# Qualcomm-AI-research/transformer-quantization

Hardware: AMD Instinct MI355X
Metric: M elems/sec fake-quant fwd (BERT-base act tensor); achieved HBM GB/s vs peak (higher is better)
Workload: dtype f32; 1 GPU; BERT-base W8A8 per-tensor asym 8-bit activation fake-quant, running-minmax calibrated, fixed-range fwd, hidden [1024,512,768] bf16 per GPU (BASELINE configs[1]); storage_dtype=bf16, parallelism=dp1 (independent shards, no data-path collective)

## Files before the change

### include/tq_hip.h

```cpp
#ifndef TQ_HIP_H
#define TQ_HIP_H

#include <stddef.h>
#include <stdint.h>

#ifdef __cplusplus
extern "C" {
#endif

#define TQ_ABI_VERSION 2

enum { TQ_F32 = 0, TQ_BF16 = 1, TQ_F16 = 2 };
enum { TQ_IDX_NONE = 0, TQ_IDX_F32 = 1, TQ_IDX_I8 = 2, TQ_IDX_U8 = 3, TQ_IDX_I16 = 4,
       TQ_IDX_I32 = 5, TQ_IDX_I8_M128 = 6  };
enum { TQ_OK = 0, TQ_EINVAL = -1, TQ_ELAUNCH = -2, TQ_EWORKSPACE = -3, TQ_EUNSUPPORTED = -4 };
enum { TQ_EST_CURRENT = 0, TQ_EST_ALL = 1, TQ_EST_RUNNING = 2 };
enum { TQ_ADA_SIGMOID = 0, TQ_ADA_HARD_SIGMOID = 1, TQ_ADA_SIGMOID_TEMP = 2 };

typedef void* tq_stream_t;

typedef struct tq_quantizer {
  const float*   delta;
  const float*   zero_float;
  const uint8_t* signed_flag;
// ... 8 lines not shown
int tq_abi_version(void);
const char* tq_last_error(void);

int tq_fake_quant_fwd(const void* x, void* y, void* idx, int idx_dtype, uint64_t n, int dtype,
                      const tq_quantizer* q, tq_stream_t stream);

typedef struct tq_fq_item {
  const void*  x;
  void*        y;
  uint64_t     n;
  tq_quantizer q;
} tq_fq_item;
int tq_fake_quant_multi_fwd(const tq_fq_item* items, uint32_t n_items, int dtype, tq_stream_t stream);

int tq_affine_fake_quant_fwd(const void* x, const float* w, const float* b, void* y,
                             int8_t* y_idx ,
                             uint64_t n, uint64_t d, int dtype, const tq_quantizer* q, tq_stream_t stream);

int tq_residual_layernorm_quant_fwd(const void* dense_out, const void* residual, void* y,
                                    int8_t* y_idx ,
                                    uint64_t rows, uint64_t d, int dtype,
                                    const tq_quantizer* q_dense, const tq_quantizer* q_sum,
                                    const float* ln_weight, const float* ln_bias, float ln_eps,
                                    const tq_quantizer* q_out, tq_stream_t stream);

int tq_residual_layernorm_quant_axis_fwd(const void* dense_out, const void* residual, void* y,
                                         int8_t* y_idx ,
                                         uint64_t rows, uint64_t d, int dtype,
                                         const tq_quantizer* q_dense, const tq_quantizer* q_sum,
                                         const float* ln_weight, const float* ln_bias, float ln_eps,
                                         const tq_quantizer* q_out, tq_stream_t stream);

int tq_residual_nonorm_quant_fwd(const void* dense_out, const void* residual, void* y, int8_t* y_idx,
                                 uint64_t rows, uint64_t d, int dtype, const tq_quantizer* q_dense,
                                 const tq_quantizer* q_sum, const float* weight, const float* bias,
                                 const tq_quantizer* q_out, tq_stream_t stream);

int tq_embeddings_layernorm_quant_fwd(const float* word_table, uint64_t word_rows, const int64_t* word_ids,
                                      const float* type_table, uint64_t type_rows, const int64_t* type_ids,
                                      const float* pos_table, uint64_t pos_rows, const int64_t* pos_ids, float* y,
                                      int8_t* y_idx , uint64_t rows, uint64_t d,
                                      const tq_quantizer* q_sum1, const tq_quantizer* q_sum2, const float* ln_weight,
                                      const float* ln_bias, float ln_eps, const tq_quantizer* q_out,
                                      int32_t* bad_ids , tq_stream_t stream);

enum { TQ_ACT_NONE = 0, TQ_ACT_RELU = 1, TQ_ACT_GELU = 2, TQ_ACT_TANH = 3 };
int tq_rowsum_i8(const int8_t* w_idx, int32_t* rowsum, uint64_t N, uint64_t K, tq_stream_t stream);
int tq_linear_i8_fwd(const int8_t* x_idx, const int8_t* w_idx, const int32_t* w_rowsum,
                     const float* bias, void* y,
                     int8_t* y_idx ,
                     int y_dtype, uint64_t M, uint64_t N, uint64_t K,
                     const float* x_delta, const float* x_zero_float, int x_n_bits, float x_eps,
                     const float* w_delta, uint64_t w_n_params, float w_eps, int activation,
                     const tq_quantizer* q_out, tq_stream_t stream);

size_t tq_act_stair_bytes(uint32_t n_bins);
int tq_act_stair_build(int activation, const tq_quantizer* q_out, uint32_t n_bins, void* table, size_t table_bytes,
                       tq_stream_t stream);
int tq_linear_i8_stair_fwd(const int8_t* x_idx, const int8_t* w_idx, const int32_t* w_rowsum,
                           const float* bias, void* y, int8_t* y_idx, int y_dtype, uint64_t M, uint64_t N, uint64_t K,
                           const float* x_delta, const float* x_zero_float, int x_n_bits, float x_eps,
                           const float* w_delta, uint64_t w_n_params, float w_eps, int activation,
                           const tq_quantizer* q_out, const void* act_stair, uint32_t stair_bins, tq_stream_t stream);

#define TQ_CLS_MAX 24
typedef struct tq_cls_table {
  uint32_t n_classes;
  uint32_t end[TQ_CLS_MAX];
  uint32_t rep[TQ_CLS_MAX];
} tq_cls_table;
int tq_linear_i8_cls_fwd(const int8_t* x_idx, const int8_t* w_idx, const int32_t* cls_rowsum, const float* bias, void* y,
                         int8_t* y_idx, int y_dtype, uint64_t M, uint64_t N, uint64_t K, const float* x_delta,
                         const float* x_zero_float, uint64_t x_n_params, int x_n_bits, float x_eps, const tq_cls_table* cls,
                         const float* w_delta, uint64_t w_n_params, float w_eps, int activation, const tq_quantizer* q_out,
                         const void* act_stair, uint32_t stair_bins, tq_stream_t stream);
uint32_t tq_linear_i8_cls_stair_bins(uint64_t M, uint64_t N, uint64_t K, uint32_t n_classes);

int tq_linear_i8_nonorm_fwd(const int8_t* x_idx, const int8_t* w_idx, const int32_t* w_rowsum, const float* bias,
                            const float* residual, const float* nn_weight, const float* nn_bias, void* y,
                            int8_t* y_idx, int y_dtype, uint64_t M, uint64_t N, uint64_t K, const float* x_delta,
                            const float* x_zero_float, int x_n_bits, float x_eps, const float* w_delta,
                            uint64_t w_n_params, float w_eps, const tq_quantizer* q_dense,
                            const tq_quantizer* q_sum, const tq_quantizer* q_out, tq_stream_t stream);
int tq_linear_i8_nonorm_grouped_fwd(const int8_t* x_idx, const int8_t* w_idx, const int32_t* w_rowsum, const float* bias,
                                    const float* nn_weight, const float* nn_bias, void* y, int8_t* y_idx, int y_dtype,
                                    uint64_t M, uint64_t N, uint64_t K, const float* x_delta, const float* x_zero_float,
                                    int x_n_bits, float x_eps, const float* w_delta , float w_eps,
                                    uint64_t n_groups , const tq_quantizer* const* q_dense,
                                    const tq_quantizer* const* q_out, tq_stream_t stream);

int tq_ffn_i8_nonorm_fwd(const int8_t* x_idx, const float* x_delta, const float* x_zero_float, int x_n_bits, float x_eps,
                         const int8_t* w1_idx, const int32_t* w1_rowsum, const float* bias1, const float* w1_delta,
                         uint64_t w1_n_params, float w1_eps, const tq_quantizer* q_mid, const int8_t* w2_idx,
                         const int32_t* w2_rowsum, const float* bias2, const float* w2_delta, uint64_t w2_n_params,
                         float w2_eps, const float* residual, const float* nn_weight, const float* nn_bias,
                         const tq_quantizer* q_dense, const tq_quantizer* q_sum, const tq_quantizer* q_out, void* y,
                         int8_t* y_idx, int y_dtype, uint64_t M, uint64_t K1, uint64_t N1, uint64_t N2,
                         tq_stream_t stream);

typedef struct tq_ffn_stage {
  const int8_t*  w1_idx;      const int32_t* w1_rowsum;  const float* bias1;   const float* w1_delta;
  uint64_t       w1_n_params; float          w1_eps;
  const tq_quantizer* q_mid;
  const int8_t*  w2_idx;      const int32_t* w2_rowsum;  const float* bias2;   const float* w2_delta;
  uint64_t       w2_n_params; float          w2_eps;
  const float*   nn_weight;   const float*   nn_bias;
  const tq_quantizer *q_dense, *q_sum, *q_out;
} tq_ffn_stage;
int tq_ffn_chain_i8_nonorm_fwd(const int8_t* x_idx, const float* x_delta, const float* x_zero_float, int x_n_bits, float x_eps,
                               const float* residual, const tq_ffn_stage* stages, uint64_t n_stages , void* y,
                               int8_t* y_idx, int y_dtype, uint64_t M, uint64_t K1, uint64_t N1, uint64_t N2,
                               tq_stream_t stream);

int tq_linear_i8_grouped_fwd(const int8_t* x_idx, const int8_t* w_idx, const int32_t* w_rowsum,
                             const float* bias, void* y, int8_t* y_idx, int y_dtype, uint64_t M,
                             uint64_t N, uint64_t K, const float* x_delta, const float* x_zero_float,
                             int x_n_bits, float x_eps, const float* w_delta, float w_eps,
                             int activation, uint64_t n_groups, const tq_quantizer* const* q_out,
                             tq_stream_t stream);

int tq_attention_i8_fwd(const int8_t* q_idx, const int8_t* k_idx, const int8_t* v_idx, float* ctx,
                        int8_t* ctx_idx, uint64_t B, uint64_t T, uint64_t H, uint64_t head_dim,
                        uint64_t qkv_row_stride ,
                        const float* mask, float denom, const tq_quantizer* q_q,
                        const tq_quantizer* q_k, const tq_quantizer* q_v, const tq_quantizer* q_scores,
                        const tq_quantizer* q_probs, const tq_quantizer* q_ctx, tq_stream_t stream);
int tq_attention_i8_strided_fwd(const int8_t* q_idx, const int8_t* k_idx, const int8_t* v_idx, float* ctx,
                                int8_t* ctx_idx, uint64_t B, uint64_t T, uint64_t H, uint64_t head_dim,
                                uint64_t qk_row_stride, uint64_t v_row_stride, const float* mask, float denom,
                                const tq_quantizer* q_q, const tq_quantizer* q_k, const tq_quantizer* q_v,
                                const tq_quantizer* q_scores, const tq_quantizer* q_probs, const tq_quantizer* q_ctx,
                                tq_stream_t stream);

int tq_scores_softmax_quant_fwd(const float* scores, float* probs, uint64_t rows, uint64_t cols,
                                const float* mask, uint64_t rows_per_mask, float denom,
                                const tq_quantizer* q_scores, const tq_quantizer* q_probs,
                                tq_stream_t stream);

size_t tq_fake_quant_bwd_workspace_bytes(uint64_t n);
size_t tq_fake_quant_bwd_params_workspace_bytes(uint64_t n, uint64_t n_params, uint64_t inner);
int tq_fake_quant_bwd(const void* x, const void* grad_y, void* grad_x, float* grad_delta,
                      float* grad_zero_float, uint64_t n, int dtype, const tq_quantizer* q,
                      void* workspace, size_t workspace_bytes, tq_stream_t stream);

size_t tq_minmax_workspace_bytes(uint64_t n, uint64_t n_params, uint64_t inner);
int tq_minmax(const void* x, uint64_t n, int dtype, uint64_t n_params, uint64_t inner,
              float* out_min, float* out_max, void* workspace, size_t workspace_bytes,
              tq_stream_t stream);

int tq_range_update(int mode, const float* new_min, const float* new_max, float* cur_min,
                    float* cur_max, uint64_t n, int initialised, double momentum,
                    uint64_t n_groups, const int64_t* order, tq_stream_t stream);

size_t tq_calibrate_workspace_bytes(uint64_t n, uint64_t n_params, uint64_t inner);
int tq_calibrate_minmax(const void* x, uint64_t n, int dtype, uint64_t n_params, uint64_t inner,
                        int mode, const float* prev_min, const float* prev_max, float* cur_min,
                        float* cur_max, double momentum, uint64_t n_groups, const int64_t* order,
                        int n_bits, int symmetric, float eps, int log_domain, float* delta,
                        float* zero_float, uint8_t* signed_flag, void* y, void* workspace,
                        size_t workspace_bytes, tq_stream_t stream);

int tq_calibrate_tensor(const void* x, uint64_t n, int dtype, int mode, const float* prev_min,
                        const float* prev_max, float* cur_min, float* cur_max, double momentum,
                        int n_bits, int symmetric, float eps, int log_domain, float* delta,
                        float* zero_float, uint8_t* signed_flag, void* y, void* workspace,
                        size_t workspace_bytes, uint32_t* counter, tq_stream_t stream);
// ... 149 lines not shown
```

### transformer-quantization_amd/csrc/tq_fused_ln.hip

```cpp
#include <algorithm>

#include "tq_device.h"
#include "tq_host.h"

namespace tq {

struct FusedQ {
  QP p;
  int on;
  float rcp;
};

__device__ __forceinline__ FusedQ make_fq(const QP& p, int on) {
  FusedQ f = {QP{1.f, 0.f, 0.f, 0.f}, on, 1.f};
  if (on) { f.p = p; f.rcp = guarded_rcp(f.p.scale); }
  return f;
}
__device__ __forceinline__ FusedQ make_fq(const tq_quantizer& q, int on) { return make_fq(on ? make_qp(q, 0) : QP{1.f, 0.f, 0.f, 0.f}, on); }

__device__ __forceinline__ float index_q(float v, const FusedQ& q) {
  return clamp_nanprop(rne_quot1(v, q.p.scale, q.rcp) + q.p.zp, q.p.lo, q.p.hi);
}

__device__ __forceinline__ float apply_q(float v, const FusedQ& q) {
  return q.on ? q_dequant(index_q(v, q), q.p) : v;
}

template <int CTRL>
__device__ __forceinline__ float dpp_f32(float v) {
  return __builtin_bit_cast(float, __builtin_amdgcn_update_dpp(0, __builtin_bit_cast(int, v), CTRL, 0xF, 0xF, true));
}
template <int LPR>
__device__ __forceinline__ float group_sum(float v) {
  static_assert(LPR >= 4 && LPR <= 64 && (LPR & (LPR - 1)) == 0, "LPR");
  v += dpp_f32<0xB1>(v);
  v += dpp_f32<0x4E>(v);
  if (LPR >= 8) v += dpp_f32<0x141>(v);
  if (LPR >= 16) v += dpp_f32<0x140>(v);
  if (LPR >= 32) v += __builtin_bit_cast(float, __builtin_amdgcn_ds_swizzle(__builtin_bit_cast(int, v), 0x401F));
  if (LPR >= 64) v += __shfl_xor(v, 32, 64);
  return v;
}

template <int LPR>
__device__ __forceinline__ float group_max(float v) {
  v = max_raw(v, dpp_f32<0xB1>(v));
  v = max_raw(v, dpp_f32<0x4E>(v));
  if (LPR >= 8) v = max_raw(v, dpp_f32<0x141>(v));
  if (LPR >= 16) v = max_raw(v, dpp_f32<0x140>(v));
  if (LPR >= 32) v = max_raw(v, __builtin_bit_cast(float, __builtin_amdgcn_ds_swizzle(__builtin_bit_cast(int, v), 0x401F)));
  if (LPR >= 64) v = max_raw(v, __shfl_xor(v, 32, 64));
  return v;
}

struct FusedF {
  QF f;
  int on;
};
__device__ __forceinline__ FusedF make_ff(const QP& p, int on) {
  FusedF r;
  r.on = on;
  r.f = make_qf(on ? p : QP{1.f, 0.f, 0.f, 1.f});
  return r;
}
__device__ __forceinline__ f32x2 apply_f2(f32x2 v, const FusedF& q) { return q.on ? qf_fake_quant2(v, q.f) : v; }

struct EmbArgs {
  const int64_t *a_rows, *a2_rows, *r_rows;
  const u32x4* a2;
  uint64_t a_n, a2_n, r_n;
  int32_t* bad;
};

template <int DT, int LPR, int NV, bool EMB>
__device__ __forceinline__ void ln_load_row(const u32x4* __restrict__ a, const u32x4* __restrict__ r, const EmbArgs& emb, int nt,
                                            int lane, uint64_t row, u32x4 (&pa)[NV], u32x4 (&pr)[NV], u32x4 (&pa2)[EMB ? NV : 1]) {
  constexpr int V = Store<DT>::kVec;
  constexpr uint32_t d = LPR * NV * V;
  if (EMB) {
    bool bad = false;
    auto pick = [&bad](const int64_t* ids, uint64_t row_, uint64_t n) {
      const int64_t id = ids[row_];
      const bool out = id < 0 || (uint64_t)id >= n;
      bad = bad || out;
      return out ? (uint64_t)0 : (uint64_t)id;
    };
    const uint64_t oa = pick(emb.a_rows, row, emb.a_n) * (d / V) + lane;
    const uint64_t o2 = pick(emb.a2_rows, row, emb.a2_n) * (d / V) + lane;
    const uint64_t orr = pick(emb.r_rows, row, emb.r_n) * (d / V) + lane;
#pragma unroll
    for (int v = 0; v < NV; ++v) { pa[v] = a[oa + v * LPR]; pa2[v] = emb.a2[o2 + v * LPR]; pr[v] = r[orr + v * LPR]; }
    if (bad) {
      const u32x4 nan4 = {0x7fc00000u, 0x7fc00000u, 0x7fc00000u, 0x7fc00000u};
#pragma unroll
      for (int v = 0; v < NV; ++v) pa[v] = nan4;
      if (lane == 0 && emb.bad) __hip_atomic_store(emb.bad, 1, __ATOMIC_RELAXED, __HIP_MEMORY_SCOPE_SYSTEM);
    }
    return;
  }
  const uint64_t o = row * (d / V) + lane;
  if (nt) {
#pragma unroll
    for (int v = 0; v < NV; ++v) { pa[v] = ld_stream(a + o + v * LPR); pr[v] = ld_stream(r + o + v * LPR); }
  } else {
#pragma unroll
    for (int v = 0; v < NV; ++v) { pa[v] = a[o + v * LPR]; pr[v] = r[o + v * LPR]; }
  }
}

struct TailQ {
  QP p1, p2, p3;
};

template <int DT, int LPR, int NV, bool IDX, bool FAST, bool ALLON, bool AFF, bool EMB>
__device__ __forceinline__ void res_ln_body(const u32x4* __restrict__ a, const u32x4* __restrict__ r,
                                            u32x4* __restrict__ y, int8_t* __restrict__ y_idx, uint64_t rows,
                                            const float* s_w, const float* s_b,
                                            float ln_eps, const TailQ& tq, int on1_, int on2_, int on3_, int nt, uint32_t iters,
                                            const EmbArgs& emb, u32x4 (&va)[NV], u32x4 (&vr)[NV], u32x4 (&va2)[EMB ? NV : 1]) {
  constexpr bool affine_only = AFF;
  const int on1 = ALLON ? 1 : on1_, on2 = ALLON ? 1 : on2_, on3 = ALLON ? 1 : on3_;
  constexpr int V = Store<DT>::kVec;
  constexpr int H = V / 2;
  constexpr int RPB = kBlock / LPR;
  constexpr uint32_t d = LPR * NV * V;
  const FusedF f1 = make_ff(tq.p1, on1), f2 = make_ff(tq.p2, on2), f3 = make_ff(tq.p3, on3);
  const FusedQ g1 = make_fq(tq.p1, on1), g2 = make_fq(tq.p2, on2), g3 = make_fq(tq.p3, on3);
  const int lane = threadIdx.x % LPR;
  const int sub = threadIdx.x / LPR;
  const float inv_d = 1.0f / (float)d;

  const uint64_t row0 = (uint64_t)blockIdx.x * RPB * iters + sub;
  u32x4 na[NV], nr[NV];
  u32x4 na2[EMB ? NV : 1];
  auto load_row = [&](uint64_t row, u32x4 (&pa)[NV], u32x4 (&pr)[NV], u32x4 (&pa2)[EMB ? NV : 1]) {
    ln_load_row<DT, LPR, NV, EMB>(a, r, emb, nt, lane, row, pa, pr, pa2);
  };
  for (uint32_t it = 0; it < iters; ++it) {
    const uint64_t row = row0 + (uint64_t)it * RPB;
    if (row >= rows) break;
    const uint64_t base = row * (d / V);
    const uint64_t nrow = row + RPB;
    if (it + 1 < iters && nrow < rows) load_row(nrow, na, nr, na2);
    f32x2 u[NV][H];
    f32x2 s2 = {0.f, 0.f}, s2b = {0.f, 0.f};
    bool lane_nan = false;
#pragma unroll
    for (int v = 0; v < NV; ++v) {
      float fa[V], fr[V];
      Store<DT>::unpack(va[v], fa);
      Store<DT>::unpack(vr[v], fr);
      if (EMB) {
        float f2[V];
        Store<DT>::unpack(va2[v], f2);
#pragma unroll
        for (int k = 0; k < V; ++k) fa[k] = fa[k] + f2[k];
      }
      if (FAST) {
        f32x2 t[H];
#pragma unroll
        for (int j = 0; j < H; ++j) t[j] = f32x2{fa[2 * j], fa[2 * j + 1]};
        if (ALLON) qf_fake_quant2_n_signed_zero<H>(t, f1.f);
        else if (f1.on) qf_fake_quant2_n<H>(t, f1.f);
#pragma unroll
        for (int j = 0; j < H; ++j) t[j] = t[j] + f32x2{fr[2 * j], fr[2 * j + 1]};
        if (ALLON) qf_fake_quant2_n_signed_zero<H>(t, f2.f);
        else if (f2.on) qf_fake_quant2_n<H>(t, f2.f);
        if (affine_only) {
#pragma unroll
          for (int j = 0; j < H; ++j) {
            t[j].x = __builtin_isunordered(fa[2 * j], fr[2 * j]) ? __builtin_nanf("") : t[j].x;
            t[j].y = __builtin_isunordered(fa[2 * j + 1], fr[2 * j + 1]) ? __builtin_nanf("") : t[j].y;
          }
        } else {
#pragma unroll
          for (int j = 0; j < H; ++j)
            lane_nan = lane_nan || __builtin_isunordered(fa[2 * j], fr[2 * j]) ||
                       __builtin_isunordered(fa[2 * j + 1], fr[2 * j + 1]);
        }
#pragma unroll
        for (int j = 0; j < H; ++j) u[v][j] = t[j];
      } else {
#pragma unroll
        for (int j = 0; j < H; ++j)
          u[v][j] = f32x2{apply_q(apply_q(fa[2 * j], g1) + fr[2 * j], g2),
                          apply_q(apply_q(fa[2 * j + 1], g1) + fr[2 * j + 1], g2)};
      }
      if (!affine_only) {
#pragma unroll
        for (int j = 0; j < H; ++j) {
          if (j & 1) s2b = s2b + u[v][j];
          else s2 = s2 + u[v][j];
        }
      }
    }
    s2 = s2 + s2b;
    float mean = 0.0f, rstd = 1.0f;
    bool row_nan = false;
    if (!affine_only) {
      mean = group_sum<LPR>(s2.x + s2.y) * inv_d;
      const f32x2 m2 = {mean, mean};
      f32x2 ssa = {0.f, 0.f}, ssb = {0.f, 0.f};
#pragma unroll
      for (int v = 0; v < NV; ++v)
#pragma unroll
        for (int j = 0; j < H; ++j) {
          const f32x2 c = u[v][j] - m2;
          if ((v * H + j) & 1) ssb = __builtin_elementwise_fma(c, c, ssb);
          else ssa = __builtin_elementwise_fma(c, c, ssa);
        }
      const f32x2 ss2 = ssa + ssb;
      rstd = 1.0f / sqrtf(group_sum<LPR>(ss2.x + ss2.y) * inv_d + ln_eps);
      if (FAST) {
        const uint64_t m = __ballot(lane_nan);
        const uint64_t grp = LPR == 64 ? ~0ull : (((1ull << (LPR % 64)) - 1) << ((threadIdx.x & 63) / LPR * LPR));
        if (m & grp) { mean = __builtin_nanf(""); row_nan = true; }
      }
    }
    const f32x2 m2 = {mean, mean}, r2 = {rstd, rstd};
    u32x4 packed[NV];
#pragma unroll
    for (int v = 0; v < NV; ++v) {
      float o[V];
      struct alignas(V) { int8_t e[V]; } oi;
      f32x2 t[H];
#pragma unroll
      for (int j = 0; j < H; ++j) {
        const uint32_t c = (v * LPR + lane) * V + 2 * j;
        const f32x2 wv = *reinterpret_cast<const f32x2*>(s_w + c), bv = *reinterpret_cast<const f32x2*>(s_b + c);
        t[j] = (u[v][j] - m2) * r2 * wv + bv;
      }
      if (f3.on) {
        if (FAST) {
          f32x2 h[H];
          qf_round2_n<H>(t, f3.f, h);
#pragma unroll
          for (int j = 0; j < H; ++j) {
            if (IDX) {
              oi.e[2 * j] = (int8_t)((int)(h[j].x + f3.f.zp) - 128);
              oi.e[2 * j + 1] = (int8_t)((int)(h[j].y + f3.f.zp) - 128);
            }
            const f32x2 yq = qf_dequant2(h[j], f3.f);
            if (affine_only) {
              t[j].x = (t[j].x != t[j].x) ? t[j].x : yq.x;
              t[j].y = (t[j].y != t[j].y) ? t[j].y : yq.y;
            } else {
              t[j] = yq;
            }
          }
        } else {
#pragma unroll
          for (int j = 0; j < H; ++j) {
            const float x0 = index_q(t[j].x, g3), x1 = index_q(t[j].y, g3);
            if (IDX) {
              oi.e[2 * j] = (int8_t)((int)x0 - 128);
              oi.e[2 * j + 1] = (int8_t)((int)x1 - 128);
            }
            t[j] = f32x2{q_dequant(x0, g3.p), q_dequant(x1, g3.p)};
          }
        }
      }
#pragma unroll
      for (int j = 0; j < H; ++j) { o[2 * j] = t[j].x; o[2 * j + 1] = t[j].y; }
      packed[v] = Store<DT>::pack(o);
      if (IDX) *reinterpret_cast<decltype(oi)*>(y_idx + (base + v * LPR + lane) * V) = oi;
    }
    if (nt) {
#pragma unroll
      for (int v = 0; v < NV; ++v) st_stream(y + base + v * LPR + lane, packed[v]);
    } else {
#pragma unroll
      for (int v = 0; v < NV; ++v) y[base + v * LPR + lane] = packed[v];
    }
    if (FAST && !affine_only && f3.on && __ballot(row_nan)) {
      if (row_nan) {
        float nanv[V];
#pragma unroll
        for (int e = 0; e < V; ++e) nanv[e] = __builtin_nanf("");
        const u32x4 pn = Store<DT>::pack(nanv);
#pragma unroll
        for (int v = 0; v < NV; ++v) y[base + v * LPR + lane] = pn;
      }
    }
#pragma unroll
    for (int v = 0; v < NV; ++v) { va[v] = na[v]; vr[v] = nr[v]; }
    if (EMB) {
#pragma unroll
      for (int v = 0; v < NV; ++v) va2[v] = na2[v];
    }
  }
}

template <int DT, int LPR, int NV, bool IDX, bool AFF, bool EMB = false>
__global__ __launch_bounds__(kBlock) void res_ln_quant_k(const u32x4* __restrict__ a, const u32x4* __restrict__ r,
                                                         u32x4* __restrict__ y, int8_t* __restrict__ y_idx, uint64_t rows,
                                                         const float* __restrict__ ln_w, const float* __restrict__ ln_b,
                                                         float ln_eps, tq_quantizer q1, tq_quantizer q2, tq_quantizer q3,
                                                         int on1, int on2, int on3, int nt, uint32_t iters, EmbArgs emb) {
  constexpr int V = Store<DT>::kVec;
  constexpr int RPB = kBlock / LPR;
  constexpr uint32_t d = LPR * NV * V;
  constexpr int NA = (d + kBlock - 1) / kBlock;
  __shared__ __attribute__((aligned(16))) float s_w[d], s_b[d];
  u32x4 va[NV], vr[NV];
  u32x4 va2[EMB ? NV : 1];
  const uint64_t row0 = (uint64_t)blockIdx.x * RPB * iters + threadIdx.x / LPR;
  if (row0 < rows) ln_load_row<DT, LPR, NV, EMB>(a, r, emb, nt, threadIdx.x % LPR, row0, va, vr, va2);
  float aw[NA], ab[NA];
#pragma unroll
  for (int i = 0; i < NA; ++i) {
    const uint32_t c = threadIdx.x + i * kBlock;
    const uint32_t cc = c < d ? c : d - 1;
    aw[i] = ln_w[cc];
    ab[i] = ln_b[cc];
  }
  QRaw w1 = load_qraw(q1, 0, ln_w), w2 = load_qraw(q2, 0, ln_w), w3 = load_qraw(q3, 0, ln_w);
  qraw_arrived(w1); qraw_arrived(w2); qraw_arrived(w3);
#pragma unroll
  for (int i = 0; i < NA; ++i) {
    const uint32_t c = threadIdx.x + i * kBlock;
    if (c < d) { s_w[c] = aw[i]; s_b[c] = ab[i]; }
  }
  __syncthreads();
  const QP none = {1.f, 0.f, 0.f, 0.f};
  const TailQ tq = {on1 ? qp_from_raw(q1, w1) : none, on2 ? qp_from_raw(q2, w2) : none, on3 ? qp_from_raw(q3, w3) : none};
  bool fast = true;
  if (on1) fast = fast && make_qf(tq.p1).ok;
  if (on2) fast = fast && make_qf(tq.p2).ok;
  if (on3) fast = fast && make_qf(tq.p3).ok;
  if (fast && on1 && on2 && on3)
    res_ln_body<DT, LPR, NV, IDX, true, true, AFF, EMB>(a, r, y, y_idx, rows, s_w, s_b, ln_eps, tq, 1, 1, 1, nt, iters, emb, va, vr, va2);
  else if (fast)
    res_ln_body<DT, LPR, NV, IDX, true, false, AFF, EMB>(a, r, y, y_idx, rows, s_w, s_b, ln_eps, tq, on1, on2, on3, nt, iters, emb, va, vr, va2);
  else
    res_ln_body<DT, LPR, NV, IDX, false, false, AFF, EMB>(a, r, y, y_idx, rows, s_w, s_b, ln_eps, tq, on1, on2, on3, nt, iters, emb, va, vr, va2);
}

template <int DT>
static int launch_res_ln(const void* a, const void* r, void* y, int8_t* y_idx, uint64_t rows, uint64_t d, const float* w, const float* b,
                         float eps, const tq_quantizer* q1, const tq_quantizer* q2, const tq_quantizer* q3, int affine_only,
                         hipStream_t st, const EmbArgs* emb_in = nullptr) {
  const EmbArgs emb = emb_in ? *emb_in : EmbArgs{};
  constexpr int V = Store<DT>::kVec;
  const tq_quantizer none{};
  const tq_quantizer &c1 = q1 ? *q1 : none, &c2 = q2 ? *q2 : none, &c3 = q3 ? *q3 : none;
  const auto av = static_cast<const u32x4*>(a);
  const auto rv = static_cast<const u32x4*>(r);
  auto yv = static_cast<u32x4*>(y);
  const uint64_t vpr = d / V;
  const int nt = rows * d * elem_size(DT) >= (64ull << 20);
#define TQ_LN_GO(LPR, NV, IDXV, AFFV)                                                                           \
  hipLaunchKernelGGL((res_ln_quant_k<DT, LPR, NV, IDXV, AFFV>), dim3(grid), dim3(kBlock), 0, st, av, rv, yv, y_idx, rows, w, b, \
                     eps, c1, c2, c3, q1 != nullptr, q2 != nullptr, q3 != nullptr, nt, iters, emb)
#define TQ_LN(LPR, NV)                                                                                          \
  if (vpr == (uint64_t)(LPR) * (NV)) {                                                                          \
    const unsigned rpb = kBlock / (LPR);                                                                        \
    const uint32_t iters = (uint32_t)std::max<int>(1, std::min<uint64_t>(tuning("TQ_TAIL_ITERS", DT == TQ_F32 ? 2 : 8), ceil_div(rows, (uint64_t)rpb * 2048))); \
    const unsigned grid = (unsigned)std::max<uint64_t>(ceil_div(rows, (uint64_t)rpb * iters), 1);               \
    if (DT == TQ_F32 && emb_in != nullptr) {                                                                    \
      if (y_idx != nullptr) hipLaunchKernelGGL((res_ln_quant_k<TQ_F32, LPR, NV, true, false, true>), dim3(grid), dim3(kBlock), 0, st, av, rv, yv, y_idx, rows, w, b, \
                                               eps, c1, c2, c3, q1 != nullptr, q2 != nullptr, q3 != nullptr, 0, iters, emb); \
      else hipLaunchKernelGGL((res_ln_quant_k<TQ_F32, LPR, NV, false, false, true>), dim3(grid), dim3(kBlock), 0, st, av, rv, yv, y_idx, rows, w, b, \
                              eps, c1, c2, c3, q1 != nullptr, q2 != nullptr, q3 != nullptr, 0, iters, emb);   \
      return check_launch("res_ln_quant_k (embeddings)");                                                       \
    }                                                                                                           \
    if (y_idx != nullptr && affine_only)      TQ_LN_GO(LPR, NV, true, true);                                    \
    else if (y_idx != nullptr)                TQ_LN_GO(LPR, NV, true, false);                                   \
    else if (affine_only)                     TQ_LN_GO(LPR, NV, false, true);                                   \
    else                                      TQ_LN_GO(LPR, NV, false, false);                                  \
    return check_launch("res_ln_quant_k");                                                                      \
  }
  TQ_LN(32, 3) TQ_LN(64, 3) TQ_LN(64, 6) TQ_LN(64, 12) TQ_LN(64, 1) TQ_LN(64, 2) TQ_LN(64, 4) TQ_LN(16, 1) TQ_LN(32, 1) TQ_LN(64, 8)
#undef TQ_LN
#undef TQ_LN_GO
  return set_error(TQ_EUNSUPPORTED, "tq_residual_layernorm_quant_fwd: row length %llu has no instantiation",
                   (unsigned long long)d);
}

constexpr uint64_t kAxisMaxD = 1024;

template <int H>
__device__ __forceinline__ void lds_pairs(const float* s, uint32_t c0, f32x2 (&o)[H]) {
#pragma unroll
  for (int k = 0; k < H / 2; ++k) {
    const f32x4 t = *reinterpret_cast<const f32x4*>(s + c0 + 4 * k);
    o[2 * k] = f32x2{t[0], t[1]};
    o[2 * k + 1] = f32x2{t[2], t[3]};
  }
}

template <int H, uint32_t D>
__device__ __forceinline__ void axq_round(const f32x2 (&x)[H], const float* tab, uint32_t c0, f32x2 (&h)[H], f32x2 (&sc)[H]) {
  f32x2 rc[H], lo[H], hi[H], xc[H], q0[H], e[H];
  lds_pairs<H>(tab, c0, sc);
  lds_pairs<H>(tab + D, c0, rc);
  lds_pairs<H>(tab + 2 * D, c0, lo);
  lds_pairs<H>(tab + 3 * D, c0, hi);
#pragma unroll
  for (int i = 0; i < H; ++i) {
    xc[i].x = __builtin_amdgcn_fmed3f(x[i].x, lo[i].x, hi[i].x);
    xc[i].y = __builtin_amdgcn_fmed3f(x[i].y, lo[i].y, hi[i].y);
  }
#pragma unroll
  for (int i = 0; i < H; ++i) q0[i] = xc[i] * rc[i];
#pragma unroll
  for (int i = 0; i < H; ++i) e[i] = __builtin_elementwise_fma(q0[i], -sc[i], xc[i]);
#pragma unroll
  for (int i = 0; i < H; ++i) q0[i] = __builtin_elementwise_fma(e[i], rc[i], q0[i]);
#pragma unroll
  for (int i = 0; i < H; ++i) h[i] = f32x2{rintf(q0[i].x), rintf(q0[i].y)};
}
template <int H, uint32_t D, bool PLUS0>
__device__ __forceinline__ void axq_fake_quant(f32x2 (&x)[H], const float* tab, uint32_t c0) {
  f32x2 h[H], sc[H];
  axq_round<H, D>(x, tab, c0, h, sc);
#pragma unroll
  for (int i = 0; i < H; ++i) x[i] = PLUS0 ? __builtin_elementwise_fma(sc[i], h[i], f32x2{0.0f, 0.0f}) : sc[i] * h[i];
}
// ... 604 lines not shown
```

### transformer-quantization_amd/csrc/tq_linear_i8.hip

```cpp
#include <algorithm>
#include <type_traits>

#include "tq_device.h"
#include "tq_host.h"

namespace tq {

typedef int v4i __attribute__((ext_vector_type(4)));

enum { ACT_NONE = 0, ACT_RELU = 1, ACT_GELU = 2, ACT_TANH = 3 };

__device__ __forceinline__ float apply_act(float v, int act) {
  switch (act) {
    case ACT_RELU: return v > 0.0f ? v : 0.0f;
    case ACT_GELU: return 0.5f * v * (1.0f + erff(v * 0.70710678118654752440f));
    case ACT_TANH: return tanhf(v);
    default: return v;
  }
}

struct LinArgs {
  const int8_t* x;
  const int8_t* w;
  const int32_t* w_rowsum;
  const float* bias;
  void* y;
  int8_t* y_idx;
  uint32_t M, N, K;
  const float* x_delta;
  const float* x_zero_float;
  float x_eps;
  int x_n_bits;
  const float* w_delta;
  uint32_t w_n_params;
  float w_eps;
  int act;
  int has_q;
  tq_quantizer q_out;
  tq_quantizer q_out1, q_out2;
  uint32_t group_cols;
  int fast_epi;
  int dbg;
  int tail;
  const float* residual;
  const float* nn_w;
  const float* nn_b;
  tq_quantizer q_t1, q_t2;
  int on_t1, on_t2;
  tq_quantizer q_t2b, q_t2c;
  int split_out;
  const float* stair;
  uint32_t stair_bins;
};

struct StairRef {
  const u32x2* tab;
  float inv_w, c0, nbm1;
};

__device__ __forceinline__ uint32_t out_group(const LinArgs& p, uint32_t n0) { return p.split_out ? n0 / p.group_cols : 0; }
__device__ __forceinline__ size_t out_at(const LinArgs& p, uint32_t g, uint32_t row, uint32_t n) {
  if (!p.split_out) return (size_t)row * p.N + n;
  return (size_t)g * p.M * p.group_cols + (size_t)row * p.group_cols + (n - g * p.group_cols);
}


template <int NP>
__device__ __forceinline__ void gelu_erf_n(f32x2 (&v)[NP]) {
  f32x2 a[NP], t[NP], q[NP];
  const f32x2 one = {1.0f, 1.0f};
  auto k2 = [](float c) { return f32x2{c, c}; };
#pragma unroll
  for (int i = 0; i < NP; ++i) {
    a[i] = v[i] * k2(0.70710678118654752440f);
    t[i] = __builtin_elementwise_abs(a[i]);
  }
#pragma unroll
  for (int i = 0; i < NP; ++i) q[i] = __builtin_elementwise_fma(t[i], k2(-4.5358574425335974e-05f), k2(0.00044550743768922985f));
#pragma unroll
  for (int i = 0; i < NP; ++i) q[i] = __builtin_elementwise_fma(t[i], q[i], k2(-0.0014894409105181694f));
#pragma unroll
  for (int i = 0; i < NP; ++i) q[i] = __builtin_elementwise_fma(t[i], q[i], k2(-0.0007746309274807572f));
#pragma unroll
  for (int i = 0; i < NP; ++i) q[i] = __builtin_elementwise_fma(t[i], q[i], k2(0.02825368195772171f));
#pragma unroll
  for (int i = 0; i < NP; ++i) q[i] = __builtin_elementwise_fma(t[i], q[i], k2(-0.14848162233829498f));
#pragma unroll
  for (int i = 0; i < NP; ++i) q[i] = __builtin_elementwise_fma(t[i], q[i], k2(-0.9184163808822632f));
#pragma unroll
  for (int i = 0; i < NP; ++i) q[i] = __builtin_elementwise_fma(t[i], q[i], k2(-1.6279085874557495f));
#pragma unroll
  for (int i = 0; i < NP; ++i) q[i] = q[i] * t[i];
#pragma unroll
  for (int i = 0; i < NP; ++i) {
    f32x2 e = {__builtin_amdgcn_exp2f(q[i].x), __builtin_amdgcn_exp2f(q[i].y)};
    e = one - e;
    f32x2 r;
    r.x = __builtin_copysignf(e.x, a[i].x);
    r.y = __builtin_copysignf(e.y, a[i].y);
    v[i] = (v[i] * k2(0.5f)) * (one + r);
  }
}

template <int YDT>
__device__ __forceinline__ void store_y4(void* y, size_t at, f32x2 lo, f32x2 hi) {
  if (YDT == TQ_F32) {
    *reinterpret_cast<f32x4*>(static_cast<float*>(y) + at) = f32x4{lo.x, lo.y, hi.x, hi.y};
  } else {
    u32x2 pk;
    pk[0] = __builtin_bit_cast(uint32_t, __builtin_convertvector(lo, bf16x2));
    pk[1] = __builtin_bit_cast(uint32_t, __builtin_convertvector(hi, bf16x2));
    *reinterpret_cast<u32x2*>(static_cast<uint16_t*>(y) + at) = pk;
  }
}

template <int WTN, int PR, int YDT>
__device__ __forceinline__ void stage_flush(const LinArgs& p, const int8_t* ystage, const int8_t* istage, uint32_t n0, uint32_t mrow0,
                                            int lane, bool want_idx) {
  constexpr int ES = YDT == TQ_F32 ? 4 : 2;
  constexpr int YP = WTN * ES + 16, IP = WTN + 16;
  const uint32_t og = out_group(p, n0);
  if (p.y != nullptr) {
    constexpr int LPR = WTN * ES / 16, RPI = 64 / LPR;
#pragma unroll
    for (int t = 0; t < (PR + RPI - 1) / RPI; ++t) {
      const int row = t * RPI + lane / LPR;
      if (RPI <= PR || row < PR) {
        const u32x4 d = *reinterpret_cast<const u32x4*>(ystage + row * YP + (lane % LPR) * 16);
        __builtin_nontemporal_store(d, reinterpret_cast<u32x4*>(static_cast<int8_t*>(p.y) +
                                                                out_at(p, og, mrow0 + row, n0) * ES + (lane % LPR) * 16));
      }
    }
  }
  if (want_idx) {
    constexpr int LPR = WTN / 16, RPI = 64 / LPR;
#pragma unroll
// ... 257 lines not shown
            const float xi = q_index(v, q2);
            oi4.e[r] = (int8_t)((int)xi - 128);
            v = q_dequant(xi, q2);
          }
        }
        o[r] = v;
      }
      if (keep != nullptr) {
        constexpr int ES = YDT == TQ_F32 ? 4 : 2, YP = NI * 16 * ES + 16, IP = NI * 16 + 16;
        const int row = j * 16 + r16, col = i * 16 + kg * 4;
        *reinterpret_cast<uint32_t*>(keep + 16 * YP + row * IP + col) = __builtin_bit_cast(uint32_t, oi4);
      } else {
        if (p.y_idx != nullptr) *reinterpret_cast<uint32_t*>(p.y_idx + at) = __builtin_bit_cast(uint32_t, oi4);
        if (p.y != nullptr) store_y4<YDT>(p.y, at, f32x2{o[0], o[1]}, f32x2{o[2], o[3]});
      }
    }
  }
}

struct EpiCtx {
  QP qo;
  QF qf, qf1, qf2;
  float sx;
  int shift;
  bool fast;
  bool stair;
  float st_inv_w, st_c0, st_nbm1;
};

struct EpiRaw {
  float dx, zx;
  QRaw qo, q1, q2;
  float st[4];
  tq_quantizer qsel;
  tq_quantizer t2sel;
};

template <bool WITH_TAIL, bool GROUPED = true>
__device__ __forceinline__ EpiRaw epilogue_fetch(const LinArgs& p, uint32_t n0) {
  EpiRaw w;
  const uint32_t grp = GROUPED ? n0 / p.group_cols : 0;
  if (GROUPED) {
#define TQ_SEL(f) w.qsel.f = grp == 0 ? p.q_out.f : (grp == 1 ? p.q_out1.f : p.q_out2.f)
    TQ_SEL(delta); TQ_SEL(zero_float); TQ_SEL(signed_flag); TQ_SEL(n_bits); TQ_SEL(symmetric); TQ_SEL(log_domain); TQ_SEL(eps);
    TQ_SEL(n_params); TQ_SEL(inner);
#undef TQ_SEL
  } else {
    w.qsel = p.q_out;
  }
  w.dx = p.x_delta[0];
  w.zx = p.x_zero_float[0];
  w.qo = load_qraw(w.qsel, 0, p.x_delta);
  w.q1 = w.q2 = w.qo;
  w.t2sel = p.q_t2;
  if (WITH_TAIL) {
    if (GROUPED && p.split_out && grp == 1) w.t2sel = p.q_t2b;
    if (GROUPED && p.split_out && grp == 2) w.t2sel = p.q_t2c;
    w.q1 = load_qraw(p.q_t1, 0, p.x_delta);
    w.q2 = load_qraw(w.t2sel, 0, p.x_delta);
  }
  w.st[0] = w.st[1] = w.st[2] = w.st[3] = 0.0f;
  if (!WITH_TAIL && p.stair != nullptr) {
#pragma unroll
    for (int i = 0; i < 4; ++i) w.st[i] = p.stair[i];
  }
  return w;
}

template <bool WITH_TAIL>
__device__ __forceinline__ void epilogue_arrived(EpiRaw& w) {
  w.dx = pinned_uniform(w.dx);
  w.zx = pinned_uniform(w.zx);
  qraw_arrived(w.qo);
  if (WITH_TAIL) { qraw_arrived(w.q1); qraw_arrived(w.q2); }
  else {
#pragma unroll
    for (int i = 0; i < 4; ++i) w.st[i] = pinned_uniform(w.st[i]);
  }
}

template <bool WITH_TAIL, bool SEL = false>
__device__ __forceinline__ EpiCtx epilogue_finish(const LinArgs& p, const EpiRaw& w) {
  EpiCtx c;
  c.sx = w.dx < p.x_eps ? p.x_eps : w.dx;
  const int zx = (int)clamp_nanprop(rintf(w.zx), 0.0f, grid_top(p.x_n_bits));
  c.shift = 128 - zx;
  c.qo = QP{1.f, 0.f, 0.f, 0.f};
  if (p.has_q) c.qo = qp_from_raw<SEL>(w.qsel, w.qo);
  c.qf = make_qf(c.qo);
  c.fast = p.act != ACT_TANH && (!p.has_q || c.qf.ok) && p.fast_epi != 0;
  c.stair = false;
  c.st_inv_w = c.st_c0 = c.st_nbm1 = 0.0f;
  if (!WITH_TAIL && p.stair != nullptr && p.has_q && c.fast) {
    c.st_inv_w = w.st[0]; c.st_c0 = w.st[1]; c.st_nbm1 = w.st[2];
    c.stair = w.st[3] == 1.0f && c.st_nbm1 == (float)(p.stair_bins - 1);
  }
  c.qf1 = c.qf2 = c.qf;
  if (WITH_TAIL) {
    c.qf1 = make_qf(p.on_t1 ? qp_from_raw<SEL>(p.q_t1, w.q1) : QP{1.f, 0.f, 0.f, 1.f});
    c.qf2 = make_qf(p.on_t2 ? qp_from_raw<SEL>(w.t2sel, w.q2) : QP{1.f, 0.f, 0.f, 1.f});
    c.fast = c.fast && p.act == ACT_NONE && c.qf1.ok && c.qf2.ok;
  }
  return c;
}

template <bool WITH_TAIL>
__device__ __forceinline__ EpiCtx epilogue_prepare(const LinArgs& p, uint32_t n0) {
  EpiRaw w = epilogue_fetch<WITH_TAIL>(p, n0);
  epilogue_arrived<WITH_TAIL>(w);
  return epilogue_finish<WITH_TAIL>(p, w);
}

template <int NI, int MI, int YDT, bool STAGED, bool WITH_TAIL, bool FLUSH = true, bool FPRE = false>
__device__ __forceinline__ void linear_epilogue(const LinArgs& p, v4i (&acc)[NI][MI], uint32_t n0, uint32_t m0, int r16,
                                                int kg, const EpiCtx& c, int8_t* stage = nullptr, const float* cst = nullptr,
                                                int cs = 2 * NI * 16, const f32x4 (*res_pre)[MI] = nullptr,
                                                const u32x2* stair_lds = nullptr) {
  static_assert(!(FPRE && WITH_TAIL), "class-ordered input grids: no fused tail");
  if (!c.fast) return linear_epilogue_generic<NI, MI, YDT, FPRE>(p, acc, n0, m0, r16, kg, c.qo, c.shift, c.sx, res_pre, FLUSH ? nullptr : stage);
  if (WITH_TAIL) {
#define TQ_EPI_T(Q, T) linear_epilogue_fast<NI, MI, YDT, ACT_NONE, Q, STAGED, T, FLUSH>(p, acc, n0, m0, r16, kg, c.qf, c.shift, c.sx, stage, cst, c.qf1, c.qf2, cs, res_pre)
    if (p.tail == 2) { if (p.has_q) TQ_EPI_T(true, 2); else TQ_EPI_T(false, 2); }
    else             { if (p.has_q) TQ_EPI_T(true, 1); else TQ_EPI_T(false, 1); }
#undef TQ_EPI_T
    return;
  }
#define TQ_EPI(A, Q) linear_epilogue_fast<NI, MI, YDT, A, Q, STAGED, 0, true, FPRE>(p, acc, n0, m0, r16, kg, c.qf, c.shift, c.sx, stage, cst, QF{}, QF{}, cs)
  if (STAGED && c.stair && stair_lds != nullptr) {
    linear_epilogue_stair<NI, MI, YDT, FPRE>(p, acc, n0, m0, r16, kg, c.qf, stage, cst, cs, StairRef{stair_lds, c.st_inv_w, c.st_c0, c.st_nbm1});
    return;
  }
  if (p.has_q) {
    if (p.act == ACT_GELU)      TQ_EPI(ACT_GELU, true);
    else if (p.act == ACT_RELU) TQ_EPI(ACT_RELU, true);
    else                        TQ_EPI(ACT_NONE, true);
  } else {
    if (p.act == ACT_GELU)      TQ_EPI(ACT_GELU, false);
    else if (p.act == ACT_RELU) TQ_EPI(ACT_RELU, false);
    else                        TQ_EPI(ACT_NONE, false);
  }
#undef TQ_EPI
}

template <int TN, int TM, int YDT, bool WITH_TAIL>
__global__ __launch_bounds__(kBlock) void linear_i8_k(LinArgs p) {
  constexpr int NI = TN / 16, MI = TM / 16;
  const int lane = threadIdx.x & 63;
  const uint32_t tiles_m = p.M / TM;
  const uint32_t tile = blockIdx.x * (kBlock / kWave) + (threadIdx.x >> 6);
  if (tile >= tiles_m * (p.N / TN)) return;
  const uint32_t n0 = (tile / tiles_m) * TN, m0 = (tile % tiles_m) * TM;

  const int r16 = lane & 15, kg = lane >> 4;
  const int8_t* wp = p.w + (size_t)(n0 + r16) * p.K + kg * 16;
  const int8_t* xp = p.x + (size_t)(m0 + r16) * p.K + kg * 16;

  v4i acc[NI][MI];
#pragma unroll
  for (int i = 0; i < NI; ++i)
#pragma unroll
    for (int j = 0; j < MI; ++j) acc[i][j] = v4i{0, 0, 0, 0};

  v4i fw[NI], fx[MI];
#pragma unroll
  for (int i = 0; i < NI; ++i) fw[i] = *reinterpret_cast<const v4i*>(wp + (size_t)i * 16 * p.K);
#pragma unroll
  for (int j = 0; j < MI; ++j) fx[j] = *reinterpret_cast<const v4i*>(xp + (size_t)j * 16 * p.K);

  for (uint32_t k = 64; k <= p.K; k += 64) {
// ... 664 lines not shown

template <auto Kernel>
static int reserve_lds(size_t bytes, const char* what) {
  static bool attr_set[64] = {};
  int dev = 0;
  if (hipGetDevice(&dev) != hipSuccess || dev < 0 || dev >= 64) dev = -1;
  if (dev >= 0 && attr_set[dev]) return TQ_OK;
  if (hipFuncSetAttribute(reinterpret_cast<const void*>(Kernel), hipFuncAttributeMaxDynamicSharedMemorySize, (int)bytes) != hipSuccess)
    return set_error(TQ_ELAUNCH, "%s: cannot reserve %zu bytes of LDS", what, bytes);
  if (dev >= 0) attr_set[dev] = true;
  return TQ_OK;
}

template <int YDT, bool WITH_TAIL>
static int launch_linear_t(const LinArgs& a, hipStream_t st) {
  if (a.K % 128 == 0 && a.M % 64 == 0 && a.N % 64 == 0 && tuning("TQ_I8_LDS", 1)) {
    const TilePlan t = tile_plan(a.M, a.N, a.K);
    const size_t room = (t.big ? 80 * 1024 : 40 * 1024) - 512 - t.base;
    LinArgs b = a;
    if (b.stair != nullptr && ((size_t)b.stair_bins * 8 > room || !tuning("TQ_I8_STAIR", 1))) b.stair = nullptr;
    const size_t lds = t.base + (b.stair != nullptr ? (size_t)b.stair_bins * 8 : 0) + (t.big ? (size_t)tuning("TQ_I8_LDS_PAD", 0) : 0);
    constexpr int kRing = 8;
    if (!t.big && b.stair == nullptr && a.K % 256 == 0 && a.K >= (uint32_t)tuning("TQ_I8_RING_MIN_K", 1024) &&
        t.grid <= (uint64_t)tuning("TQ_I8_RING_MAX_GRID", 256)) {
      constexpr auto k = linear_i8_lds_k<32, YDT, WITH_TAIL, kRing>;
      const size_t ring_lds = (size_t)kRing * 2 * 64 * 128 + 5 * 64 * 4;
      if (int e = reserve_lds<k>(ring_lds, "linear_i8_lds_k (ring)")) return e;
      hipLaunchKernelGGL(k, dim3((unsigned)t.grid), dim3(kBlock), ring_lds, st, b);
      return check_launch("linear_i8_lds_k (ring)");
    }
    if (!t.big && b.stair == nullptr && t.grid <= (uint64_t)tuning("TQ_I8_SMALL_MAX_GRID", 256)) {
      const uint64_t grid32 = (uint64_t)(a.M / 32) * (a.N / 32);
      const size_t lds32 = 2 * 2 * 32 * 128 + 5 * 32 * 4;
      hipLaunchKernelGGL((linear_i8_lds_k<16, YDT, WITH_TAIL>), dim3((unsigned)grid32), dim3(kBlock), lds32, st, b);
      return check_launch("linear_i8_lds_k (32 x 32 tiles)");
    }
    if (t.big) hipLaunchKernelGGL((linear_i8_lds_k<64, YDT, WITH_TAIL>), dim3((unsigned)t.grid), dim3(kBlock), lds, st, b);
    else       hipLaunchKernelGGL((linear_i8_lds_k<32, YDT, WITH_TAIL>), dim3((unsigned)t.grid), dim3(kBlock), lds, st, b);
    return check_launch("linear_i8_lds_k");
  }
  const unsigned grid = (unsigned)ceil_div((uint64_t)(a.M / 32) * (a.N / 32), kBlock / kWave);
  hipLaunchKernelGGL((linear_i8_k<32, 32, YDT, WITH_TAIL>), dim3(grid), dim3(kBlock), 0, st, a);
  return check_launch("linear_i8_k");
}

constexpr size_t kClsLds64 = 52 * 1024;
struct ClsLds {
  size_t base;
  size_t cap;
};
static ClsLds cls_lds(const TilePlan& t, uint32_t n_classes) {
  return {t.base + 2 * TQ_CLS_MAX * 4 + (size_t)n_classes * t.bt * 4, (t.big ? 80 * 1024 : kClsLds64) - 512};
}

template <int YDT>
static int launch_linear_cls(LinArgs a, const ClsArgs& ct, hipStream_t st) {
  a.fast_epi = tuning("TQ_I8_FAST_EPI", 1);
  a.dbg = 0;
  const TilePlan t = tile_plan(a.M, a.N, a.K);
  const ClsLds c = cls_lds(t, ct.n);
  if (c.base > c.cap) return set_error(TQ_EINVAL, "tq_linear_i8_cls_fwd: %u classes do not fit the LDS of a block", ct.n);
  if (a.stair != nullptr && (size_t)a.stair_bins * 8 > c.cap - c.base)
    return set_error(TQ_EINVAL, "tq_linear_i8_cls_fwd: a staircase of %u bins does not fit beside %u classes", a.stair_bins, ct.n);
  if (a.stair != nullptr && !tuning("TQ_I8_STAIR", 1)) a.stair = nullptr;
  const size_t lds = c.base + (a.stair != nullptr ? (size_t)a.stair_bins * 8 : 0);
  if (t.big) {
    hipLaunchKernelGGL((linear_i8_cls_k<64, YDT>), dim3((unsigned)t.grid), dim3(kBlock), lds, st, a, ct);
  } else {
    constexpr auto k = linear_i8_cls_k<32, YDT>;
    if (int e = reserve_lds<k>(kClsLds64, "linear_i8_cls_k")) return e;
    hipLaunchKernelGGL(k, dim3((unsigned)t.grid), dim3(kBlock), lds, st, a, ct);
  }
  return check_launch("linear_i8_cls_k");
}

static int launch_linear(LinArgs a, int y_dtype, tq_stream_t stream) {
  a.fast_epi = tuning("TQ_I8_FAST_EPI", 1);
  a.dbg = tuning("TQ_I8_DBG", 0);
  hipStream_t st = static_cast<hipStream_t>(stream);
  if (y_dtype == TQ_F32) return a.tail ? launch_linear_t<TQ_F32, true>(a, st) : launch_linear_t<TQ_F32, false>(a, st);
  return a.tail ? launch_linear_t<TQ_BF16, true>(a, st) : launch_linear_t<TQ_BF16, false>(a, st);
}

struct LinShape {
  uint32_t mn, k;
  const char* rule;
};
constexpr LinShape kAnyShape{32, 64, "M,N % 32, K % 64"};
constexpr LinShape kTiledShape{64, 128, "M, N % 64, K % 128"};
constexpr LinShape kGroupedShape{64, 128, "M % 64, K % 128"};

static int lin_args(LinArgs& a, const char* who, const LinShape& s, const int8_t* x, const int8_t* w, const int32_t* w_rowsum,
                    const float* bias, void* y, int8_t* y_idx, bool need_y, int y_dtype, uint64_t M, uint64_t N, uint64_t K,
                    const float* x_delta, const float* x_zero_float, int x_n_bits, float x_eps, const float* w_delta,
                    uint64_t w_n_params, float w_eps, int act) {
  TQ_REQUIRE(x && w && w_rowsum && (need_y ? y != nullptr : y || y_idx) && x_delta && x_zero_float && w_delta, "%s: NULL pointer", who);
  TQ_REQUIRE(y_dtype == TQ_F32 || y_dtype == TQ_BF16, "%s: y dtype must be fp32 or bf16", who);
  TQ_REQUIRE(M % s.mn == 0 && N % s.mn == 0 && K % s.k == 0 && K >= s.k && K <= 16384 && M < (1u << 31) && N < (1u << 31),
             "%s: unsupported shape M=%llu N=%llu K=%llu (%s)", who, (unsigned long long)M, (unsigned long long)N,
             (unsigned long long)K, s.rule);
  TQ_REQUIRE(x_n_bits >= 1 && x_n_bits <= 8, "%s: input quantizer must have <= 8 bits", who);
  TQ_REQUIRE(w_n_params == 1 || w_n_params == N, "%s: weight scales must be per-tensor or per-output-channel", who);
  TQ_REQUIRE(act >= ACT_NONE && act <= ACT_TANH, "%s: unknown activation %d", who, act);
  TQ_REQUIRE(aligned16(x) && aligned16(w) && (y == nullptr || aligned16(y)), "%s: 16-byte alignment required", who);
  a.x = x; a.w = w; a.w_rowsum = w_rowsum; a.bias = bias; a.y = y; a.y_idx = y_idx;
  a.M = (uint32_t)M; a.N = (uint32_t)N; a.K = (uint32_t)K;
  a.x_delta = x_delta; a.x_zero_float = x_zero_float; a.x_eps = x_eps; a.x_n_bits = x_n_bits;
  a.w_delta = w_delta; a.w_n_params = (uint32_t)w_n_params; a.w_eps = w_eps; a.act = act;
  a.group_cols = (uint32_t)N;
  return TQ_OK;
}

static int check_y_idx(const char* who, const int8_t* y_idx, const tq_quantizer* q, bool groups = false) {
  if (y_idx == nullptr || (q != nullptr && !q->symmetric && q->n_bits <= 8)) return TQ_OK;
  return set_error(TQ_EINVAL, groups ? "%s: y_idx needs asymmetric <= 8-bit output quantizers"
                                     : "%s: y_idx needs an asymmetric <= 8-bit output quantizer", who);
}

static int quantizer_slot(const char* who, const char* what, const tq_quantizer* q, uint64_t n, tq_quantizer& slot, int& on) {
  on = q != nullptr;
  if (q == nullptr) return TQ_OK;
  if (int e = check_quantizer(q, n, who)) return e;
  TQ_REQUIRE(q->n_params == 1, "%s: per-tensor %s only", who, what);
  slot = *q;
  return TQ_OK;
}

static int nonorm_quantizers(LinArgs& a, const char* who, uint64_t n, const tq_quantizer* q_dense, const tq_quantizer* q_sum,
                             const tq_quantizer* q_out) {
  if (int e = quantizer_slot(who, "quantizers", q_dense, n, a.q_out, a.has_q)) return e;
  if (int e = quantizer_slot(who, "quantizers", q_sum, n, a.q_t1, a.on_t1)) return e;
  return quantizer_slot(who, "quantizers", q_out, n, a.q_t2, a.on_t2);
}

static int lin_out(LinArgs& a, const char* who, const tq_quantizer* q_out, const void* act_stair, uint32_t stair_bins) {
  TQ_REQUIRE(act_stair == nullptr || (q_out != nullptr && stair_bins >= 64 && stair_bins <= 2048 && aligned16(act_stair)),
             "%s: the staircase needs an output quantizer, 64..2048 bins and 16-byte alignment", who);
  if (int e = check_y_idx(who, a.y_idx, q_out)) return e;
  if (int e = quantizer_slot(who, "output quantizer", q_out, (uint64_t)a.M * a.N, a.q_out, a.has_q)) return e;
  a.stair = static_cast<const float*>(act_stair);
  a.stair_bins = stair_bins;
  return TQ_OK;
}

}

using namespace tq;

extern "C" int tq_rowsum_i8(const int8_t* w_idx, int32_t* rowsum, uint64_t N, uint64_t K, tq_stream_t stream) {
  TQ_REQUIRE(w_idx && rowsum && N >= 1 && K >= 1, "tq_rowsum_i8: bad argument");
  hipLaunchKernelGGL(rowsum_i8_k, dim3((unsigned)ceil_div(N, kBlock / kWave)), dim3(kBlock), 0,
                     static_cast<hipStream_t>(stream), w_idx, rowsum, (uint32_t)N, (uint32_t)K);
  return check_launch("rowsum_i8_k");
}

extern "C" int tq_linear_i8_grouped_fwd(const int8_t* x_idx, const int8_t* w_idx, const int32_t* w_rowsum,
                                        const float* bias, void* y, int8_t* y_idx, int y_dtype, uint64_t M, uint64_t N,
                                        uint64_t K, const float* x_delta, const float* x_zero_float, int x_n_bits,
                                        float x_eps, const float* w_delta, float w_eps, int activation,
                                        uint64_t n_groups, const tq_quantizer* const* q_out, tq_stream_t stream) {
  const char* who = "tq_linear_i8_grouped_fwd";
  if (M == 0 || N == 0) return TQ_OK;
  TQ_REQUIRE(q_out != nullptr, "%s: NULL pointer", who);
  TQ_REQUIRE(y != nullptr || y_idx != nullptr, "%s: no output requested", who);
  TQ_REQUIRE(n_groups >= 1 && n_groups <= 3 && N % n_groups == 0 && (N / n_groups) % 64 == 0,
             "%s: 1..3 groups of a multiple of 64 output features", who);
  LinArgs a{};
  if (int e = lin_args(a, who, kGroupedShape, x_idx, w_idx, w_rowsum, bias, y, y_idx, false, y_dtype, M, N, K, x_delta,
                       x_zero_float, x_n_bits, x_eps, w_delta, N, w_eps, activation))
    return e;
  a.group_cols = (uint32_t)(N / n_groups);
  tq_quantizer* slots[3] = {&a.q_out, &a.q_out1, &a.q_out2};
  for (uint64_t g = 0; g < n_groups; ++g) {
    TQ_REQUIRE(q_out[g] != nullptr, "%s: every group needs an output quantizer", who);
    if (int e = quantizer_slot(who, "output quantizers", q_out[g], M * N, *slots[g], a.has_q)) return e;
    if (int e = check_y_idx(who, y_idx, q_out[g], true)) return e;
  }
  return launch_linear(a, y_dtype, stream);
}

extern "C" int tq_linear_i8_fwd(const int8_t* x_idx, const int8_t* w_idx, const int32_t* w_rowsum, const float* bias,
                                void* y, int8_t* y_idx, int y_dtype, uint64_t M, uint64_t N, uint64_t K, const float* x_delta,
                                const float* x_zero_float, int x_n_bits, float x_eps, const float* w_delta,
                                uint64_t w_n_params, float w_eps, int activation, const tq_quantizer* q_out,
                                tq_stream_t stream) {
  return tq_linear_i8_stair_fwd(x_idx, w_idx, w_rowsum, bias, y, y_idx, y_dtype, M, N, K, x_delta, x_zero_float, x_n_bits, x_eps,
                                w_delta, w_n_params, w_eps, activation, q_out, nullptr, 0, stream);
}

extern "C" int tq_linear_i8_stair_fwd(const int8_t* x_idx, const int8_t* w_idx, const int32_t* w_rowsum, const float* bias,
                                      void* y, int8_t* y_idx, int y_dtype, uint64_t M, uint64_t N, uint64_t K,
                                      const float* x_delta, const float* x_zero_float, int x_n_bits, float x_eps,
                                      const float* w_delta, uint64_t w_n_params, float w_eps, int activation,
                                      const tq_quantizer* q_out, const void* act_stair, uint32_t stair_bins,
                                      tq_stream_t stream) {
  const char* who = "tq_linear_i8_stair_fwd";
  if (M == 0 || N == 0) return TQ_OK;
  LinArgs a{};
  if (int e = lin_args(a, who, kAnyShape, x_idx, w_idx, w_rowsum, bias, y, y_idx, false, y_dtype, M, N, K, x_delta, x_zero_float,
                       x_n_bits, x_eps, w_delta, w_n_params, w_eps, activation))
    return e;
  if (int e = lin_out(a, who, q_out, act_stair, stair_bins)) return e;
  return launch_linear(a, y_dtype, stream);
}

extern "C" int tq_linear_i8_cls_fwd(const int8_t* x_idx, const int8_t* w_idx, const int32_t* cls_rowsum, const float* bias, void* y,
                                    int8_t* y_idx, int y_dtype, uint64_t M, uint64_t N, uint64_t K, const float* x_delta,
                                    const float* x_zero_float, uint64_t x_n_params, int x_n_bits, float x_eps,
                                    const tq_cls_table* cls, const float* w_delta, uint64_t w_n_params, float w_eps, int activation,
// ... 213 lines not shown
```

### transformer-quantization_amd/quantization/_hip.py

```python
import ctypes as C
import os

import torch

_HERE = os.path.dirname(os.path.abspath(__file__))
LIB_PATH = os.environ.get('TQ_LIB_PATH') or os.path.join(os.path.dirname(_HERE), 'lib', 'libtq_hip.so')

TQ_F32, TQ_BF16, TQ_F16 = 0, 1, 2
IDX_NONE, IDX_F32, IDX_I8, IDX_U8, IDX_I16, IDX_I32, IDX_I8_M128 = range(7)
ACT_NONE, ACT_RELU, ACT_GELU, ACT_TANH = range(4)
EST_CURRENT, EST_ALL, EST_RUNNING = 0, 1, 2
ADA_SIGMOID, ADA_HARD_SIGMOID, ADA_SIGMOID_TEMP = 0, 1, 2

_DTYPES = {torch.float32: TQ_F32, torch.bfloat16: TQ_BF16, torch.float16: TQ_F16}
_IDX_DTYPES = {torch.float32: IDX_F32, torch.int8: IDX_I8, torch.uint8: IDX_U8,
               torch.int16: IDX_I16, torch.int32: IDX_I32}


class TQError(RuntimeError):
    pass


class tq_quantizer(C.Structure):
    _fields_ = [('delta', C.c_void_p), ('zero_float', C.c_void_p), ('signed_flag', C.c_void_p),
                ('n_bits', C.c_int32), ('symmetric', C.c_int32), ('log_domain', C.c_int32),
                ('eps', C.c_float), ('n_params', C.c_uint64), ('inner', C.c_uint64)]


class tq_fq_item(C.Structure):
    _fields_ = [('x', C.c_void_p), ('y', C.c_void_p), ('n', C.c_uint64), ('q', tq_quantizer)]


CLS_MAX = 24


class tq_cls_table(C.Structure):
    _fields_ = [('n_classes', C.c_uint32), ('end', C.c_uint32 * CLS_MAX), ('rep', C.c_uint32 * CLS_MAX)]


class tq_quantizer_f64(C.Structure):
    _fields_ = [('delta', C.c_void_p), ('zero_float', C.c_void_p), ('signed_flag', C.c_void_p),
                ('n_bits', C.c_int32), ('symmetric', C.c_int32), ('log_domain', C.c_int32),
                ('reserved', C.c_int32), ('eps', C.c_double), ('n_params', C.c_uint64), ('inner', C.c_uint64)]


_u64, _vp, _int, _sz, _f, _d = C.c_uint64, C.c_void_p, C.c_int, C.c_size_t, C.c_float, C.c_double
_QP = C.POINTER(tq_quantizer)


class tq_ffn_stage(C.Structure):
    _fields_ = [('w1_idx', C.c_void_p), ('w1_rowsum', C.c_void_p), ('bias1', C.c_void_p), ('w1_delta', C.c_void_p),
                ('w1_n_params', C.c_uint64), ('w1_eps', C.c_float), ('q_mid', _QP),
                ('w2_idx', C.c_void_p), ('w2_rowsum', C.c_void_p), ('bias2', C.c_void_p), ('w2_delta', C.c_void_p),
                ('w2_n_params', C.c_uint64), ('w2_eps', C.c_float),
                ('nn_weight', C.c_void_p), ('nn_bias', C.c_void_p), ('q_dense', _QP), ('q_sum', _QP), ('q_out', _QP)]
_QPD = C.POINTER(tq_quantizer_f64)


ABI_VERSION = 2

SIGNATURES = {
    'tq_fake_quant_fwd_f64': (_int, [_vp, _vp, _vp, _u64, _QPD, _vp]),
    'tq_fake_quant_bwd_f64_workspace_bytes': (_sz, [_u64, _u64, _u64]),
    'tq_fake_quant_bwd_f64': (_int, [_vp, _vp, _vp, _vp, _vp, _u64, _QPD, _vp, _sz, _vp]),
    'tq_minmax_f64_workspace_bytes': (_sz, [_u64, _u64, _u64]),
    'tq_minmax_f64': (_int, [_vp, _u64, _u64, _u64, _vp, _vp, _vp, _sz, _vp]),
    'tq_range_update_f64': (_int, [_int, _vp, _vp, _vp, _vp, _u64, _int, _d, _u64, _vp, _vp]),
    'tq_axis_ranges_f64': (_int, [_vp, _vp, _vp, _u64, _int, _vp]),
    'tq_set_range_asym_f64': (_int, [_vp, _vp, _u64, _int, _d, _int, _vp, _vp, _vp]),
    'tq_set_range_sym_f64': (_int, [_vp, _vp, _u64, _int, _d, _int, _vp, _vp, _vp]),
    'tq_mse_candidates_f64': (_int, [_vp, _u64, _u64, _vp, _u64, _int, _vp, _vp]),
    'tq_abi_version': (_int, []),
    'tq_last_error': (C.c_char_p, []),
    'tq_fake_quant_fwd': (_int, [_vp, _vp, _vp, _int, _u64, _int, _QP, _vp]),
    'tq_fake_quant_multi_fwd': (_int, [C.POINTER(tq_fq_item), C.c_uint32, _int, _vp]),
    'tq_affine_fake_quant_fwd': (_int, [_vp, _vp, _vp, _vp, _vp, _u64, _u64, _int, _QP, _vp]),
    'tq_residual_layernorm_quant_fwd': (_int, [_vp, _vp, _vp, _vp, _u64, _u64, _int, _QP, _QP, _vp, _vp, _f, _QP, _vp]),
    'tq_residual_layernorm_quant_axis_fwd': (_int, [_vp, _vp, _vp, _vp, _u64, _u64, _int, _QP, _QP, _vp, _vp, _f, _QP, _vp]),
    'tq_residual_nonorm_quant_fwd': (_int, [_vp, _vp, _vp, _vp, _u64, _u64, _int, _QP, _QP, _vp, _vp, _QP, _vp]),
    'tq_embeddings_layernorm_quant_fwd': (_int, [_vp, _u64, _vp, _vp, _u64, _vp, _vp, _u64, _vp, _vp, _vp, _u64, _u64, _QP, _QP,
                                                _vp, _vp, C.c_float, _QP, _vp, _vp]),
    'tq_attention_i8_fwd': (_int, [_vp, _vp, _vp, _vp, _vp, _u64, _u64, _u64, _u64, _u64, _vp, _f, _QP, _QP, _QP, _QP, _QP, _QP, _vp]),
    'tq_attention_i8_strided_fwd': (_int, [_vp, _vp, _vp, _vp, _vp, _u64, _u64, _u64, _u64, _u64, _u64, _vp, _f, _QP, _QP, _QP, _QP,
                                           _QP, _QP, _vp]),
    'tq_linear_i8_grouped_fwd': (_int, [_vp, _vp, _vp, _vp, _vp, _vp, _int, _u64, _u64, _u64, _vp, _vp, _int, _f, _vp, _f, _int,
                                        _u64, C.POINTER(_QP), _vp]),
    'tq_scores_softmax_quant_fwd': (_int, [_vp, _vp, _u64, _u64, _vp, _u64, _f, _QP, _QP, _vp]),
    'tq_rowsum_i8': (_int, [_vp, _vp, _u64, _u64, _vp]),
    'tq_ffn_i8_nonorm_fwd': (_int, [_vp, _vp, _vp, _int, _f, _vp, _vp, _vp, _vp, _u64, _f, _QP, _vp, _vp, _vp, _vp, _u64, _f,
                                    _vp, _vp, _vp, _QP, _QP, _QP, _vp, _vp, _int, _u64, _u64, _u64, _u64, _vp]),
    'tq_linear_i8_nonorm_fwd': (_int, [_vp, _vp, _vp, _vp, _vp, _vp, _vp, _vp, _vp, _int, _u64, _u64, _u64, _vp, _vp, _int, _f,
                                       _vp, _u64, _f, _QP, _QP, _QP, _vp]),
    'tq_ffn_chain_i8_nonorm_fwd': (_int, [_vp, _vp, _vp, _int, _f, _vp, _vp, _u64, _vp, _vp, _int, _u64, _u64, _u64, _u64, _vp]),
    'tq_linear_i8_nonorm_grouped_fwd': (_int, [_vp, _vp, _vp, _vp, _vp, _vp, _vp, _vp, _int, _u64, _u64, _u64, _vp, _vp, _int, _f, _vp,
                                               _f, _u64, C.POINTER(_QP), C.POINTER(_QP), _vp]),
    'tq_linear_i8_fwd': (_int, [_vp, _vp, _vp, _vp, _vp, _vp, _int, _u64, _u64, _u64, _vp, _vp, _int, _f, _vp, _u64, _f,
                                _int, _QP, _vp]),
    'tq_linear_i8_stair_fwd': (_int, [_vp, _vp, _vp, _vp, _vp, _vp, _int, _u64, _u64, _u64, _vp, _vp, _int, _f, _vp, _u64, _f,
                                      _int, _QP, _vp, C.c_uint32, _vp]),
    'tq_linear_i8_cls_fwd': (_int, [_vp, _vp, _vp, _vp, _vp, _vp, _int, _u64, _u64, _u64, _vp, _vp, _u64, _int, _f,
                                    C.POINTER(tq_cls_table), _vp, _u64, _f, _int, _QP, _vp, C.c_uint32, _vp]),
    'tq_linear_i8_cls_stair_bins': (C.c_uint32, [_u64, _u64, _u64, C.c_uint32]),
    'tq_act_stair_bytes': (_sz, [C.c_uint32]),
    'tq_act_stair_build': (_int, [_int, _QP, C.c_uint32, _vp, _sz, _vp]),
    'tq_fake_quant_bwd_workspace_bytes': (_sz, [_u64]),
    'tq_fake_quant_bwd_params_workspace_bytes': (_sz, [_u64, _u64, _u64]),
    'tq_fake_quant_bwd': (_int, [_vp, _vp, _vp, _vp, _vp, _u64, _int, _QP, _vp, _sz, _vp]),
    'tq_minmax_workspace_bytes': (_sz, [_u64, _u64, _u64]),
    'tq_minmax': (_int, [_vp, _u64, _int, _u64, _u64, _vp, _vp, _vp, _sz, _vp]),
    'tq_calibrate_workspace_bytes': (_sz, [_u64, _u64, _u64]),
    'tq_calibrate_minmax': (_int, [_vp, _u64, _int, _u64, _u64, _int, _vp, _vp, _vp, _vp, _d, _u64, _vp, _int,
                                   _int, _f, _int, _vp, _vp, _vp, _vp, _vp, _sz, _vp]),
    'tq_calibrate_tensor': (_int, [_vp, _u64, _int, _int, _vp, _vp, _vp, _vp, _d, _int, _int, _f, _int, _vp, _vp, _vp,
                                   _vp, _vp, _sz, _vp, _vp]),
    'tq_calibrate_stats': (_int, [_vp, _u64, _int, _u64, _u64, _vp, _vp, _sz, _vp, _vp]),
    'tq_calibrate_apply': (_int, [_vp, _vp, _u64, _int, _u64, _u64, _int, _vp, _vp, _vp, _vp, _d, _u64, _vp, _int, _int, _f,
                                  _int, _vp, _vp, _vp, _vp, _vp]),
    'tq_mailbox_bytes': (_sz, []),
    'tq_mailbox_max_floats': (_sz, []),
    'tq_mailbox_handle_bytes': (_sz, []),
    'tq_mailbox_alloc': (_int, [C.POINTER(_vp), _vp]),
    'tq_mailbox_open': (_int, [_vp, C.POINTER(_vp)]),
    'tq_mailbox_close': (_int, [_vp]),
    'tq_mailbox_free': (_int, [_vp]),
    'tq_mailbox_allreduce_max': (_int, [_vp, _u64, _vp, _vp, C.c_uint32, C.c_uint32, _vp, C.c_uint32, _vp]),
    'tq_calibrate_minmax_mailbox': (_int, [_vp, _u64, _int, _u64, _u64, _int, _vp, _vp, _vp, _vp, _d, _u64, _vp, _int, _int, _f,
                                           _int, _vp, _vp, _vp, _vp, _vp, _sz, _vp, _vp, _vp, C.c_uint32, C.c_uint32, _vp,
                                           C.c_uint32, _vp]),
    'tq_order_stats_workspace_bytes': (_sz, [_u64, C.c_uint32]),
    'tq_order_stats': (_int, [_vp, _u64, _u64, _int, C.POINTER(_u64), C.c_uint32, _vp, _vp, _sz, _vp]),
    'tq_comm_unique_id_bytes': (_sz, []),
    'tq_comm_load': (_int, [C.c_char_p]),
    'tq_comm_version': (_int, []),
    'tq_comm_get_unique_id': (_int, [_vp]),
    'tq_comm_init': (_int, [_vp, _int, _int, C.POINTER(_vp)]),
    'tq_comm_destroy': (_int, [_vp]),
    'tq_comm_abort': (_int, [_vp]),
    'tq_comm_rank_world': (_int, [_vp, C.POINTER(_int), C.POINTER(_int)]),
    'tq_comm_allreduce': (_int, [_vp, _vp, _u64, _int, _int, _vp]),
    'tq_comm_broadcast': (_int, [_vp, _vp, _u64, _int, _int, _vp]),
    'tq_calibrate_minmax_rccl': (_int, [_vp, _u64, _int, _u64, _u64, _int, _vp, _vp, _vp, _vp, _d, _u64, _vp, _int, _int, _f,
                                        _int, _vp, _vp, _vp, _vp, _vp, _sz, _vp, _vp, _vp]),
    'tq_range_update': (_int, [_int, _vp, _vp, _vp, _vp, _u64, _int, _d, _u64, _vp, _vp]),
    'tq_axis_ranges': (_int, [_vp, _vp, _vp, _u64, _int, _vp]),
    'tq_set_range_asym': (_int, [_vp, _vp, _u64, _int, _f, _int, _vp, _vp, _vp]),
    'tq_set_range_sym': (_int, [_vp, _vp, _u64, _int, _f, _int, _vp, _vp, _vp]),
    'tq_mse_workspace_bytes': (_sz, [_u64, _u64, _u64]),
    'tq_mse_candidates': (_int, [_vp, _u64, _u64, _int, _vp, _u64, _vp, _vp, _sz, _vp]),
    'tq_mse_candidates_grouped': (_int, [_vp, _u64, _u64, _u64, _int, _vp, _u64, _vp, _vp, _sz, _vp]),
    'tq_mse_ordered_workspace_bytes': (_sz, [_u64, _u64, _u64]),
    'tq_mse_candidates_ordered': (_int, [_vp, _u64, _u64, _int, _vp, _u64, _int, _vp, _vp, _vp, _sz, _vp]),
    'tq_xent_candidates': (_int, [_vp, _u64, _u64, _vp, _u64, _vp, _vp]),
    'tq_argmin_select': (_int, [_vp, _u64, _u64, _vp, _vp, _vp, _vp, _vp, _vp]),
    'tq_adaround_fwd': (_int, [_vp, _vp, _vp, _u64, _QP, _int, _int, _f, _vp]),
    'tq_adaround_init_alpha': (_int, [_vp, _vp, _u64, _QP, _int, _f, _vp]),
    'tq_adaround_bwd': (_int, [_vp, _vp, _vp, _vp, _u64, _QP, _int, _f, _vp]),
    'tq_adaround_bwd_adam_sched': (_int, [_vp, _vp, _vp, _vp, _vp, _u64, _QP, _int, _f, _vp, _f, _f, _f, _f, _vp]),
    'tq_adaround_bwd_adam': (_int, [_vp, _vp, _vp, _vp, _vp, _vp, _u64, _QP, _int, _f, _f, _f, _f,
                                    _f, _f, _f, _int, _vp]),
    'tq_adaround_reg': (_int, [_vp, _u64, _int, _f, _f, _f, _vp, _vp, _sz, _vp]),
    'tq_reduce_workspace_bytes': (_sz, [_u64]),
    'tq_recon_loss': (_int, [_vp, _vp, _u64, _u64, _u64, _vp, _vp, _sz, _vp]),
}

_lib = None


def load_library(path=None):
    global _lib
    if _lib is not None and path is None:
        return _lib
    p = path or LIB_PATH
    if not os.path.exists(p):
        raise TQError(
            f'{p} not found: build it with `python transformer-quantization_amd/build.py` '
# ... 42 lines not shown


def _check(rc, lib):
    if rc != 0:
        raise TQError(f'libtq_hip: {lib.tq_last_error().decode()} (code {rc})')


def _ptr(t):
    return None if t is None else t.data_ptr()


_raw_stream = getattr(torch._C, '_cuda_getCurrentRawStream', None)


def _stream():
    if _raw_stream is not None:
        return _raw_stream(torch.cuda.current_device())
    return torch.cuda.current_stream().cuda_stream


def _need_device(t, what):
    if not t.is_cuda:
        raise TQError(f'{what}: tensor lives on {t.device}; the fake-quant path only runs on a '
                      'ROCm device (no CPU fallback)')


def _need_f32(what, *tensors):
    for t in tensors:
        if t is not None and t.dtype != torch.float32:
            raise TQError(f'{what}: fp32 tensors required, got {t.dtype} (call .float() on the layer first)')


def _dtype_code(t, what):
    try:
        return _DTYPES[t.dtype]
    except KeyError:
        hint = ' -- float64 (--double) runs the layered quantizer path only' if t.dtype == torch.float64 else ''
        raise TQError(f'{what}: dtype {t.dtype} not supported (fp32 / bf16 / fp16){hint}') from None


def _device_guarded(fn):
    import functools

    _Tensor, _cur = torch.Tensor, torch.cuda.current_device

    @functools.wraps(fn)
    def wrapper(self, *args, **kwargs):
        idx = -1
        for a in args:
            if isinstance(a, _Tensor):
                i = a.get_device()
                if i < 0:
                    continue
                if idx < 0:
                    idx = i
                elif i != idx:
                    raise TQError(f'{fn.__name__}: operands live on different devices (cuda:{idx} and cuda:{i})')
        if idx < 0:
            for a in args:
                if isinstance(a, (tuple, list)):
                    for b in a:
                        if isinstance(b, _Tensor) and b.get_device() >= 0:
                            idx = b.get_device()
                            break
                    if idx >= 0:
                        break
        if idx < 0 or idx == _cur():
            return fn(self, *args, **kwargs)
        with torch.cuda.device(idx):
            return fn(self, *args, **kwargs)
    return wrapper


class HipBackend:

    name = 'hip'

    def __init__(self):
        self.lib = load_library()
        self._ws = {}
        self._qdesc_cache = {}
        self._ws_bytes = {}
        self._counters = {}
        self._calib_tensor_addr = None

    def _workspace(self, device, nbytes):
        key = (device.index, _stream())
        ws = self._ws.get(key)
        if ws is None or ws.numel() < nbytes:
            ws = torch.empty(max(int(nbytes), 1 << 16), dtype=torch.uint8, device=device)
            self._ws[key] = ws
        return ws

    def _calib_ws_bytes(self, n, n_params, inner):
        key = (n, n_params, inner)
        v = self._ws_bytes.get(key)
        if v is None:
            if len(self._ws_bytes) > 4096:
                self._ws_bytes.clear()
            v = self._ws_bytes[key] = self.lib.tq_calibrate_workspace_bytes(n, n_params, inner)
        return v

    def to_device_f32(self, v, like=None):
        if torch.is_tensor(v):
            if v.is_cuda:
                return v if v.dtype == torch.float32 else v.float()
            dev = like.device if (like is not None and like.is_cuda) else torch.device(
                'cuda', torch.cuda.current_device())
            return v.detach().to(device=dev, dtype=torch.float32)
        dev = like.device if (like is not None and like.is_cuda) else torch.device(
            'cuda', torch.cuda.current_device())
        return torch.tensor(v, dtype=torch.float64).float().to(dev)

    def _qdesc(self, delta, zero_float, signed, n_bits, symmetric, log_domain, eps, n_params, inner):
        key = (None if delta is None else delta.data_ptr(), None if zero_float is None else zero_float.data_ptr(),
               None if signed is None else signed.data_ptr(), n_bits, symmetric, log_domain, eps, n_params, inner)
        cache = self._qdesc_cache
        d = cache.get(key)
        if d is None:
            if len(cache) > 8192:
                cache.clear()
            d = cache[key] = tq_quantizer(key[0], key[1], key[2], int(n_bits), int(bool(symmetric)),
                                          int(bool(log_domain)), float(eps), int(n_params), int(inner))
        return d

    @staticmethod
    def _as_f64(t, like):
        if t is None:
            return None
        t = t.detach()
        if t.dtype != torch.float64 or t.device != like.device:
            t = t.to(device=like.device, dtype=torch.float64)
        return t.contiguous()

    def _qdesc_f64(self, delta, zero_float, signed, n_bits, symmetric, log_domain, eps, n_params, inner):
        return tq_quantizer_f64(_ptr(delta), _ptr(zero_float), _ptr(signed), int(n_bits), int(bool(symmetric)),
                                int(bool(log_domain)), 0, float(eps), int(n_params), int(inner))

    def _fake_quant_f64(self, x, delta, zero_float, signed, n_bits, symmetric, log_domain, eps, n_params, inner,
                        want_y, want_idx):
        x = x.contiguous()
        d, z = self._as_f64(delta, x), self._as_f64(zero_float, x)
        y = torch.empty_like(x) if want_y else None
        idx = torch.empty_like(x) if want_idx else None
        q = self._qdesc_f64(d, z, signed, n_bits, symmetric, log_domain, eps, n_params, inner)
        rc = self.lib.tq_fake_quant_fwd_f64(_ptr(x), _ptr(y), _ptr(idx), x.numel(), C.byref(q), _stream())
        _check(rc, self.lib)
        return y, idx

    def fake_quant(self, x, delta, zero_float, signed, n_bits, symmetric, log_domain, eps,
                   n_params, inner, want_y=True, idx_dtype=None):
        _need_device(x, 'fake_quant')
        if x.dtype == torch.float64:
            if idx_dtype not in (None, torch.float32, torch.float64):
                raise TQError('fake_quant: float64 tensors emit float64 indices only')
            return self._fake_quant_f64(x, delta, zero_float, signed, n_bits, symmetric, log_domain, eps, n_params,
                                        inner, want_y, idx_dtype is not None)
        x = x.contiguous()
        y = torch.empty_like(x) if want_y else None
        idx = torch.empty(x.shape, dtype=idx_dtype, device=x.device) if idx_dtype is not None else None
        q = self._qdesc(delta, zero_float, signed, n_bits, symmetric, log_domain, eps, n_params, inner)
        rc = self.lib.tq_fake_quant_fwd(_ptr(x), _ptr(y), _ptr(idx),
                                        _IDX_DTYPES[idx_dtype] if idx_dtype is not None else IDX_NONE,
                                        x.numel(), _dtype_code(x, 'fake_quant'), C.byref(q), _stream())
        _check(rc, self.lib)
        return y, idx
# ... 190 lines not shown

    def rowsum_i8(self, w_idx):
        out = torch.empty(w_idx.shape[0], dtype=torch.int32, device=w_idx.device)
        rc = self.lib.tq_rowsum_i8(_ptr(w_idx), _ptr(out), w_idx.shape[0], w_idx.shape[1], _stream())
        _check(rc, self.lib)
        return out

    STAIR_BINS = 768
    STAIR_BINS_BIG = 1536

    def stair_bins_for(self, M, N):
        big = M % 128 == 0 and N % 128 == 0 and (M // 128) * (N // 128) >= 1024
        return self.STAIR_BINS_BIG if big else self.STAIR_BINS

    def act_stair(self, activation, q_out, n_bins=None):
        n_bins = int(n_bins or self.STAIR_BINS)
        dev = q_out[0].device
        table = torch.empty(self.lib.tq_act_stair_bytes(n_bins), dtype=torch.uint8, device=dev)
        qd = self._qdesc(*q_out, 1, 1)
        rc = self.lib.tq_act_stair_build(int(activation), C.byref(qd), n_bins, table.data_ptr(), table.numel(), _stream())
        _check(rc, self.lib)
        return table, n_bins

    def linear_i8(self, x_idx, w_idx, w_rowsum, bias, x_q, w_delta, w_eps, activation, q_out, out_dtype,
                  want_idx=False, want_y=True, stair=None):
        K = x_idx.shape[-1]
        M = x_idx.numel() // K
        N = w_idx.shape[0]
        shape = x_idx.shape[:-1] + (N,)
        y = torch.empty(shape, dtype=out_dtype, device=x_idx.device) if want_y else None
        y_idx = torch.empty(shape, dtype=torch.int8, device=x_idx.device) if want_idx else None
        qd = None if q_out is None else self._qdesc(*q_out, 1, 1)
        rc = self.lib.tq_linear_i8_stair_fwd(
            _ptr(x_idx), _ptr(w_idx), _ptr(w_rowsum), _ptr(bias), _ptr(y), _ptr(y_idx), _DTYPES[out_dtype], M, N, K,
            _ptr(x_q[0]), _ptr(x_q[1]), int(x_q[2]), float(x_q[3]), _ptr(w_delta), w_delta.numel(),
            float(w_eps), int(activation), None if qd is None else C.byref(qd),
            None if stair is None else stair[0].data_ptr(), 0 if stair is None else int(stair[1]), _stream())
        _check(rc, self.lib)
        return (y, y_idx) if want_idx else y

    def cls_table(self, ends, reps):
        t = tq_cls_table()
        t.n_classes = len(ends)
        for c, (e, r) in enumerate(zip(ends, reps)):
            t.end[c], t.rep[c] = int(e), int(r)
        return t

    def cls_stair_bins_for(self, M, N, K, n_classes):
        return self.lib.tq_linear_i8_cls_stair_bins(M, N, K, n_classes) or None

    def linear_i8_cls(self, x_idx, w_idx, cls_rowsum, bias, x_q, cls, w_delta, w_eps, activation, q_out, out_dtype,
                      want_idx=False, want_y=True, stair=None):
        K = x_idx.shape[-1]
        M = x_idx.numel() // K
        N = w_idx.shape[0]
        shape = x_idx.shape[:-1] + (N,)
        y = torch.empty(shape, dtype=out_dtype, device=x_idx.device) if want_y else None
        y_idx = torch.empty(shape, dtype=torch.int8, device=x_idx.device) if want_idx else None
        qd = None if q_out is None else self._qdesc(*q_out, 1, 1)
        rc = self.lib.tq_linear_i8_cls_fwd(
            _ptr(x_idx), _ptr(w_idx), _ptr(cls_rowsum), _ptr(bias), _ptr(y), _ptr(y_idx), _DTYPES[out_dtype], M, N, K,
            _ptr(x_q[0]), _ptr(x_q[1]), x_q[0].numel(), int(x_q[2]), float(x_q[3]), C.byref(cls), _ptr(w_delta),
            w_delta.numel(), float(w_eps), int(activation), None if qd is None else C.byref(qd),
            None if stair is None else stair[0].data_ptr(), 0 if stair is None else int(stair[1]), _stream())
        _check(rc, self.lib)
        return (y, y_idx) if want_idx else y

    def linear_i8_nonorm(self, x_idx, w_idx, w_rowsum, bias, residual, nn_w, nn_b, x_q, w_delta, w_eps, q_dense, q_sum,
                         q_out, out_dtype, want_idx=False):
        K = x_idx.shape[-1]
        M = x_idx.numel() // K
        N = w_idx.shape[0]
        y = torch.empty(x_idx.shape[:-1] + (N,), dtype=out_dtype, device=x_idx.device)
        y_idx = torch.empty(y.shape, dtype=torch.int8, device=y.device) if want_idx else None
        descs = [None if q is None else self._qdesc(*q, 1, 1) for q in (q_dense, q_sum, q_out)]
        refs = [None if d is None else C.byref(d) for d in descs]
        if residual is not None:
            residual = residual.detach().float().contiguous()
        rc = self.lib.tq_linear_i8_nonorm_fwd(
            _ptr(x_idx), _ptr(w_idx), _ptr(w_rowsum), _ptr(bias), _ptr(residual), _ptr(nn_w.detach().float().contiguous()),
            _ptr(nn_b.detach().float().contiguous()), _ptr(y), _ptr(y_idx), _DTYPES[out_dtype], M, N, K, _ptr(x_q[0]),
            _ptr(x_q[1]), int(x_q[2]), float(x_q[3]), _ptr(w_delta), w_delta.numel(), float(w_eps), refs[0], refs[1],
            refs[2], _stream())
        _check(rc, self.lib)
        return (y, y_idx) if want_idx else y

    def linear_i8_nonorm_grouped(self, x_idx, w_idx, w_rowsum, bias, nn_w, nn_b, x_q, w_delta_rows, w_eps, q_dense, q_out,
                                 out_dtype, want_idx=False, n_groups=2):
        K = x_idx.shape[-1]
        M = x_idx.numel() // K
        N = w_idx.shape[0]
        G = int(n_groups)
        y = torch.empty((G,) + tuple(x_idx.shape[:-1]) + (N // G,), dtype=out_dtype, device=x_idx.device)
        y_idx = torch.empty(y.shape, dtype=torch.int8, device=y.device) if want_idx else None

        def arr(qs):
            if qs is None:
                return None, None
            descs = [self._qdesc(*q, 1, 1) for q in qs]
            return descs, C.cast((C.POINTER(tq_quantizer) * G)(*[C.pointer(d) for d in descs]), C.POINTER(_QP))
        keep_d, a_d = arr(q_dense)
        keep_o, a_o = arr(q_out)
        rc = self.lib.tq_linear_i8_nonorm_grouped_fwd(
            _ptr(x_idx), _ptr(w_idx), _ptr(w_rowsum), _ptr(bias), _ptr(nn_w), _ptr(nn_b), _ptr(y), _ptr(y_idx),
            _DTYPES[out_dtype], M, N, K, _ptr(x_q[0]), _ptr(x_q[1]), int(x_q[2]), float(x_q[3]), _ptr(w_delta_rows),
            float(w_eps), G, a_d, a_o, _stream())
        _check(rc, self.lib)
        ys = [y[g] for g in range(G)]
        return (ys, [y_idx[g] for g in range(G)]) if want_idx else ys

    def ffn_chain_i8_nonorm(self, x_idx, x_q, residual, stages, out_dtype, want_idx=False):
        K1 = x_idx.shape[-1]
        M = x_idx.numel() // K1
        N1, N2 = stages[0]['w1_idx'].shape[0], stages[0]['w2_idx'].shape[0]
        y = torch.empty(x_idx.shape[:-1] + (N2,), dtype=out_dtype, device=x_idx.device)
        y_idx = torch.empty(y.shape, dtype=torch.int8, device=y.device) if want_idx else None
        keep = []
        arr = (tq_ffn_stage * len(stages))()
        for a, g in zip(arr, stages):
            def qp(q):
                if q is None:
                    return None
                d = self._qdesc(*q, 1, 1)
                keep.append(d)
                return C.pointer(d)

            def f32(t):
                t = t.detach().float().contiguous()
                keep.append(t)
                return t.data_ptr()
            a.w1_idx, a.w1_rowsum, a.bias1 = _ptr(g['w1_idx']), _ptr(g['w1_rowsum']), _ptr(g['bias1'])
            a.w1_delta, a.w1_n_params, a.w1_eps = _ptr(g['w1_delta']), g['w1_delta'].numel(), float(g['w1_eps'])
            a.q_mid = qp(g['q_mid'])
            a.w2_idx, a.w2_rowsum, a.bias2 = _ptr(g['w2_idx']), _ptr(g['w2_rowsum']), _ptr(g['bias2'])
            a.w2_delta, a.w2_n_params, a.w2_eps = _ptr(g['w2_delta']), g['w2_delta'].numel(), float(g['w2_eps'])
            a.nn_weight, a.nn_bias = f32(g['nn_w']), f32(g['nn_b'])
            a.q_dense, a.q_sum, a.q_out = qp(g['q_dense']), qp(g['q_sum']), qp(g['q_out'])
        res = residual.detach().float().contiguous()
        rc = self.lib.tq_ffn_chain_i8_nonorm_fwd(_ptr(x_idx), _ptr(x_q[0]), _ptr(x_q[1]), int(x_q[2]), float(x_q[3]), _ptr(res),
                                                 C.cast(arr, C.c_void_p), len(stages), _ptr(y), _ptr(y_idx), _DTYPES[out_dtype],
                                                 M, K1, N1, N2, _stream())
        _check(rc, self.lib)
        return (y, y_idx) if want_idx else y

    FFN_SHAPES = {(128, 512, 128)}

    def ffn_i8_nonorm(self, x_idx, x_q, w1_idx, w1_rowsum, bias1, w1_delta, w1_eps, q_mid, w2_idx, w2_rowsum, bias2, w2_delta,
                      w2_eps, residual, nn_w, nn_b, q_dense, q_sum, q_out, out_dtype, want_idx=False):
        K1 = x_idx.shape[-1]
        M = x_idx.numel() // K1
        N1, N2 = w1_idx.shape[0], w2_idx.shape[0]
        y = torch.empty(x_idx.shape[:-1] + (N2,), dtype=out_dtype, device=x_idx.device)
        y_idx = torch.empty(y.shape, dtype=torch.int8, device=y.device) if want_idx else None
        descs = [None if q is None else self._qdesc(*q, 1, 1) for q in (q_mid, q_dense, q_sum, q_out)]
        refs = [None if d is None else C.byref(d) for d in descs]
        rc = self.lib.tq_ffn_i8_nonorm_fwd(
            _ptr(x_idx), _ptr(x_q[0]), _ptr(x_q[1]), int(x_q[2]), float(x_q[3]), _ptr(w1_idx), _ptr(w1_rowsum), _ptr(bias1),
            _ptr(w1_delta), w1_delta.numel(), float(w1_eps), refs[0], _ptr(w2_idx), _ptr(w2_rowsum), _ptr(bias2),
            _ptr(w2_delta), w2_delta.numel(), float(w2_eps), _ptr(residual.detach().float().contiguous()),
            _ptr(nn_w.detach().float().contiguous()), _ptr(nn_b.detach().float().contiguous()), refs[1], refs[2], refs[3],
            _ptr(y), _ptr(y_idx), _DTYPES[out_dtype], M, K1, N1, N2, _stream())
        _check(rc, self.lib)
        return (y, y_idx) if want_idx else y

    def fake_quant_bwd(self, x, grad_y, delta, zero_float, signed, n_bits, symmetric, log_domain, eps,
                       n_params, inner, param_grads=False):
# ... 526 lines not shown
```

### transformer-quantization_amd/quantization/fused.py

```python
import torch

from quantization import _hip
from quantization import options
from quantization import provenance
from quantization.base_quantized_classes import FP32Acts
from quantization.quantization_manager import QuantizationManager, Qstates, _GLOBAL_FWD_HOOKS, _GLOBAL_FWD_PRE_HOOKS


def _fixed_per_tensor(enabled, mgr):
    if not enabled or isinstance(mgr, FP32Acts):
        return 'off'
    if not isinstance(mgr, QuantizationManager) or mgr.state != Qstates.fix_ranges:
        return 'no'
    q = mgr.quantizer
    if mgr._forward_hooks or mgr._forward_pre_hooks or q._forward_hooks or q._forward_pre_hooks:
        return 'no'
    if not q.is_initialized or q._delta.numel() != 1:
        return 'no'
    return (q._delta, q._zero_float, getattr(q, '_signed', None), q.n_bits, q.symmetric,
            q.scale_domain == 'log', q.eps)


def _fixed_along_last(enabled, mgr, d):
    q7 = _fixed_per_tensor(enabled, mgr)
    if q7 != 'no':
        return q7
    if not isinstance(mgr, QuantizationManager) or mgr.state != Qstates.fix_ranges:
        return 'no'
    q = mgr.quantizer
    if mgr._forward_hooks or mgr._forward_pre_hooks or q._forward_hooks or q._forward_pre_hooks:
        return 'no'
    delta = getattr(q, '_delta', None)
    if (not q.is_initialized or delta is None or d <= 1 or delta.numel() != d or delta.shape[-1] != d
            or delta.requires_grad or delta.dtype != torch.float32 or getattr(q, 'per_channel', False)
            or q.scale_domain != 'linear'):
        return 'no'
    zf = getattr(q, '_zero_float', None)
    if not q.symmetric and (zf is None or zf.numel() != d or zf.shape[-1] != d or zf.dtype != torch.float32):
        return 'no'
    return (delta.reshape(-1), None if zf is None else zf.reshape(-1), getattr(q, '_signed', None), q.n_bits, q.symmetric,
            False, q.eps)


def _per_column(*qs):
    return any(isinstance(q, tuple) and q[0].numel() != 1 for q in qs)


def _axis_tail_ok(d, dtype):
    vec = 4 if dtype == torch.float32 else 8
    return (hasattr(_hip.backend(), 'residual_layernorm_quant_axis') and dtype in (torch.float32, torch.bfloat16, torch.float16)
            and d <= _AXIS_MAX_D and d % vec == 0 and d // vec in _LN_VECTORS)


def _hooked(*modules):
    if _GLOBAL_FWD_HOOKS or _GLOBAL_FWD_PRE_HOOKS:
        return True
    return any(m is not None and isinstance(m, torch.nn.Module) and (m._forward_hooks or m._forward_pre_hooks)
               for m in modules)


hooked = _hooked


def residual_layernorm_quant(dense, res_quantizer, layer_norm, x, residual, _gemm=None):
    if _gemm is not None:
        x = _gemm
    d_out = dense.out_features if hasattr(dense, 'out_features') else x.shape[-1]
    q1 = _fixed_along_last(dense._quant_a and dense.activation_function is None, dense.activation_quantizer, d_out)
    q2 = _fixed_along_last(getattr(res_quantizer, '_quant_a', False),
                           getattr(res_quantizer, 'activation_quantizer', res_quantizer), d_out)
    q3 = _fixed_along_last(layer_norm._quant_a and layer_norm.activation_function is None,
                           layer_norm.activation_quantizer, d_out)
    from quantization.autoquant_utils import QuantNoNorm
    is_nonorm = isinstance(layer_norm, QuantNoNorm)
    axis = _per_column(q1, q2, q3)
    if axis and (is_nonorm or not _axis_tail_ok(d_out, x.dtype)
                 or tuple(getattr(layer_norm, 'normalized_shape', ())) != (d_out,)):
        q1 = 'no'
    fusable = ('no' not in (q1, q2, q3) and dense.activation_function is None
               and layer_norm.activation_function is None and _hip.on_device(x) and x.dtype != torch.float64
               and not (torch.is_grad_enabled() and (x.requires_grad or residual.requires_grad))
               and (is_nonorm or len(layer_norm.normalized_shape) == 1)
               and dense.activation_save_target is None and layer_norm.activation_save_target is None
               and not _hooked(dense, res_quantizer, layer_norm))
    if not fusable:
        if _gemm is not None:
            raise RuntimeError('residual_layernorm_quant: pre-computed GEMM handed to a tail that is not fusable')
        return layer_norm(res_quantizer(dense(x) + residual))
    if is_nonorm and _gemm is None:
        y = _linear_nonorm_i8(dense, layer_norm, x, residual, q1, q2, q3)
        if y is not None:
            return y
    gemm = _gemm
    if gemm is None and options.int8_active() and hasattr(dense, '_int8_forward'):
        gemm = dense._int8_forward(x, with_output_quantizer=False)
    if gemm is None:
        w, b = dense.get_params()
        gemm = dense.run_forward(x, w, b)
    if is_nonorm:
        ln_w, ln_b = layer_norm.quantized_params()
    else:
        ln_w, ln_b = layer_norm.get_params()
    arg = lambda q: None if q == 'off' else q
    oq = layer_norm.activation_quantizer.quantizer if q3 != 'off' else None
    want_idx = (options.int8_active() and oq is not None and not oq.symmetric and oq.n_bits <= 8
                and gemm.dtype == torch.float32)
    tail = _hip.backend().residual_layernorm_quant_axis if axis else _hip.backend().residual_layernorm_quant
    out = tail(gemm, residual, arg(q1), arg(q2), ln_w, ln_b, None if is_nonorm else layer_norm.eps, arg(q3),
               want_idx=want_idx)
    y = out[0] if want_idx else out
    if oq is not None:
        provenance.tag(y, oq, out[1] if want_idx else None)
    return y


_LN_VECTORS = (16, 32, 64, 96, 128, 192, 256, 384, 512, 768)
_AXIS_MAX_D = 1024


def embeddings_layernorm_quant(word_emb, type_emb, pos_emb, sum1, sum2, layer_norm, input_ids, type_ids, pos_ids):
    from quantization.autoquant_utils import QuantEmbedding, QuantLayerNorm
    be = _hip.backend()
    embs = (word_emb, type_emb, pos_emb)
    if (not hasattr(be, 'embeddings_layernorm_quant') or not _hip.on_device(input_ids) or input_ids.dim() != 2
            or input_ids.dtype != torch.int64 or type(layer_norm) is not QuantLayerNorm
            or layer_norm.activation_function is not None or len(layer_norm.normalized_shape) != 1
            or layer_norm.activation_save_target is not None or layer_norm.training
            or _needs_autograd(word_emb, type_emb, pos_emb, layer_norm) or _hooked(*embs, sum1, sum2, layer_norm)):
        return None
    for e in embs:
        if (type(e) is not QuantEmbedding or e.training or e.max_norm is not None or e.activation_save_target is not None
                or not isinstance(e.activation_quantizer, FP32Acts) or _hooked(e._modules.get('weight_quantizer'))):
            return None
    q1 = _fixed_per_tensor(getattr(sum1, '_quant_a', False), getattr(sum1, 'activation_quantizer', sum1))
    q2 = _fixed_per_tensor(getattr(sum2, '_quant_a', False), getattr(sum2, 'activation_quantizer', sum2))
    q3 = _fixed_per_tensor(layer_norm._quant_a, layer_norm.activation_quantizer)
    if 'no' in (q1, q2, q3):
        return None
    tables = [e.get_params()[0] for e in embs]
    d = tables[0].shape[-1]
    if (any(t.dtype != torch.float32 or t.shape[-1] != d or not _hip.on_device(t) for t in tables) or d % 4
            or d // 4 not in _LN_VECTORS):
        return None
    B, T = input_ids.shape
    if pos_ids.shape[-1] != T or type_ids.shape != input_ids.shape:
        return None
    pos_full = pos_ids.expand(B, T) if pos_ids.shape[0] != B else pos_ids
    ln_w, ln_b = layer_norm.get_params()
    arg = lambda q: None if q == 'off' else q
    oq = layer_norm.activation_quantizer.quantizer if q3 != 'off' else None
    want_idx = options.int8_active() and oq is not None and not oq.symmetric and oq.n_bits <= 8
    out = be.embeddings_layernorm_quant(tables[0], input_ids, tables[1], type_ids, tables[2], pos_full, arg(q1), arg(q2),
                                        ln_w, ln_b, layer_norm.eps, arg(q3), want_idx=want_idx)
    y = (out[0] if want_idx else out).view(B, T, d)
    if oq is not None:
        provenance.tag(y, oq, out[1].view(B, T, d) if want_idx else None)
    return y


def quantized_bert_ffn(intermediate, dense, res_quantizer, layer_norm, x, residual):
    def separate():
        return residual_layernorm_quant(dense, res_quantizer, layer_norm, intermediate(x), residual)

    if (not options.int8_active() or not hasattr(intermediate, '_int8_plan') or not hasattr(dense, '_int8_plan_from')
            or not _hip.on_device(x) or x.dtype != torch.float32 or dense.activation_function is not None
            or _needs_autograd(intermediate, dense, layer_norm, x, residual)
            or _hooked(intermediate, dense, res_quantizer, layer_norm)):
        return separate()
    from quantization.autoquant_utils import QuantNoNorm
    d_out = dense.out_features
    q1 = _fixed_along_last(dense._quant_a, dense.activation_quantizer, d_out)
    q2 = _fixed_along_last(getattr(res_quantizer, '_quant_a', False), getattr(res_quantizer, 'activation_quantizer', res_quantizer),
                           d_out)
    q3 = _fixed_along_last(layer_norm._quant_a and layer_norm.activation_function is None, layer_norm.activation_quantizer, d_out)
    if ('no' in (q1, q2, q3) or isinstance(layer_norm, QuantNoNorm) or layer_norm.activation_function is not None
            or len(layer_norm.normalized_shape) != 1 or dense.activation_save_target is not None
            or layer_norm.activation_save_target is not None or intermediate.activation_save_target is not None
            or residual.dtype != torch.float32
            or (_per_column(q1, q2, q3) and (not _axis_tail_ok(d_out, torch.float32)
                                             or tuple(layer_norm.normalized_shape) != (d_out,)))):
        return separate()
    plan1 = intermediate._int8_plan(x, with_output_quantizer=True, peg=True)
    if plan1 is None or plan1[2] is None or plan1[2][4] or plan1[2][5] or plan1[2][3] > 8:
        return separate()
    mid_q = intermediate.activation_quantizer.quantizer
    M = x.numel() // intermediate.in_features
    plan2 = dense._int8_plan_from(mid_q, M, with_output_quantizer=False)
    if plan2 is None or not dense._int8_weights()[2]:
        return separate()
    mid_idx = intermediate._int8_compute(x, plan1, index_only=True)
    if mid_idx is None:
        return separate()
    gemm = dense._int8_compute(None, plan2, x_idx=mid_idx)
    if gemm is None:
        return separate()
    return residual_layernorm_quant(dense, res_quantizer, layer_norm, None, residual, _gemm=gemm)


def _needs_autograd(*modules_and_tensors):
    if not torch.is_grad_enabled():
        return False
    for m in modules_and_tensors:
        if m is None:
            continue
        if torch.is_tensor(m):
            if m.requires_grad:
                return True
        elif any(p.requires_grad for p in m.parameters()):
            return True
    return False


def _linear_nonorm_i8(dense, layer_norm, x, residual, q1, q2, q3):
    if not options.int8_active() or not hasattr(dense, '_int8_plan') or (residual is not None and (
            residual.dtype != torch.float32 or not _hip.on_device(residual))) or _needs_autograd(dense, layer_norm, x, residual):
        return None
    plan = dense._int8_plan(x, with_output_quantizer=False)
    if plan is None or plan[1] != _hip.ACT_NONE:
        return None
    ops = dense._int8_operands(x, plan)
    if ops is None:
        return None
    from quantization.autoquant_utils import INT8_STATS
    arg = lambda q: None if q == 'off' else q
    ln_w, ln_b = layer_norm.quantized_params()
    oq = layer_norm.activation_quantizer.quantizer if q3 != 'off' else None
    want_idx = oq is not None and not oq.symmetric and oq.n_bits <= 8
    INT8_STATS['kernel_calls'] += 1
    out = _hip.backend().linear_i8_nonorm(ops[0], ops[1], ops[2], ops[3], residual, ln_w, ln_b, ops[4], ops[5], ops[6],
                                          arg(q1), arg(q2), arg(q3), torch.float32, want_idx=want_idx)
    y = out[0] if want_idx else out
    if oq is not None:
        provenance.tag(y, oq, out[1] if want_idx else None)
    return y


def linear_nonorm_quant(dense, layer_norm, x):
    from quantization.autoquant_utils import QuantNoNorm
    if (isinstance(layer_norm, QuantNoNorm) and _hip.on_device(x) and x.dtype == torch.float32
            and dense.activation_function is None and layer_norm.activation_function is None
            and dense.activation_save_target is None and layer_norm.activation_save_target is None
            and not _needs_autograd(dense, layer_norm, x) and not _hooked(dense, layer_norm)):
        q1 = _fixed_per_tensor(dense._quant_a, dense.activation_quantizer)
        q3 = _fixed_per_tensor(layer_norm._quant_a, layer_norm.activation_quantizer)
        if 'no' not in (q1, q3):
            y = _linear_nonorm_i8(dense, layer_norm, x, None, q1, 'off', q3)
            if y is not None:
                return y
    return layer_norm(dense(x))


def linear_nonorm_quant_pair(dense_a, layer_norm_a, dense_b, layer_norm_b, x, value=None):
    from quantization.autoquant_utils import QuantLinear, QuantNoNorm, INT8_STATS, _fixed_per_tensor_manager
    be = _hip.backend()
    pairs = ((dense_a, layer_norm_a), (dense_b, layer_norm_b))
    if (not options.int8_active() or not hasattr(be, 'linear_i8_nonorm_grouped') or not _hip.on_device(x)
            or x.dtype != torch.float32 or _needs_autograd(dense_a, layer_norm_a, dense_b, layer_norm_b, x)
            or _hooked(dense_a, layer_norm_a, dense_b, layer_norm_b)):
        return None
    K = x.shape[-1]
    M = x.numel() // K
    N = dense_a.out_features
    if M % 64 or K % 128 or K > 16384 or N % 64 or dense_b.out_features != N:
        return None
    q_dense, q_out, plans = [], [], []
    for d, ln in pairs:
        if (type(d) is not QuantLinear or type(ln) is not QuantNoNorm or d.training or ln.training or d.in_features != K
                or d.activation_function is not None or ln.activation_function is not None
                or d.activation_save_target is not None or ln.activation_save_target is not None
                or not hasattr(d, '_int8_plan') or _hooked(getattr(d, 'weight_quantizer', None))):
            return None
        q1 = _fixed_per_tensor(d._quant_a, d.activation_quantizer)
        q3 = _fixed_per_tensor(ln._quant_a, ln.activation_quantizer)
        if 'no' in (q1, q3):
            return None
        plan = d._int8_plan(x, with_output_quantizer=False)
        if plan is None or plan[1] != _hip.ACT_NONE:
            return None
        q_dense.append(q1)
        q_out.append(q3)
        plans.append(plan)
    if ((q_dense[0] == 'off') != (q_dense[1] == 'off') or (q_out[0] == 'off') != (q_out[1] == 'off')
            or dense_a.weight_quantizer.quantizer.eps != dense_b.weight_quantizer.quantizer.eps):
        return None
    oqs = [ln.activation_quantizer.quantizer if q != 'off' else None for (_, ln), q in zip(pairs, q_out)]
    layers = [dense_a, dense_b]
    if (value is not None and q_dense[0] != 'off' and q_out[0] != 'off' and type(value) is QuantLinear and not value.training
            and value.in_features == K and value.out_features == N and value.activation_function is None
            and value.activation_save_target is None and hasattr(value, '_int8_plan') and value._quant_a
            and _fixed_per_tensor_manager(value.activation_quantizer) and not _needs_autograd(value)
            and not _hooked(value, getattr(value, 'weight_quantizer', None))
            and value.weight_quantizer.quantizer.eps == dense_a.weight_quantizer.quantizer.eps):
        vq = value.activation_quantizer.quantizer
# ... 324 lines not shown
```

### transformer-quantization_amd/quantization/options.py

```python
import torch

INT8_LINEAR = 'auto'

INT8_CALIBRATION = True
INT8_CALIBRATION_MIN_MACS = 1 << 33

INT8_ACT_STAIR = True

LOCKSTEP_WEIGHT_SEARCH = True

INPLACE_CALIBRATION_STATE = False

GRAPH_ADAROUND = True

CACHE_EPOCH = 0


def int8_active():
    m = INT8_LINEAR
    if not m:
        return False
    if torch.is_inference_mode_enabled():
        return False
    if m is True:
        return True
    return not torch.is_grad_enabled()


def fuse_on(flag, module=None, probe=None):
    if flag is None:
        if not int8_active() or (module is not None and module.training):
            return False
        if probe is not None:
            mgr = probe._modules.get('activation_quantizer')
            state = getattr(mgr, 'state', None)
            return state is None or state.name == 'fix_ranges'
        return True
    return bool(flag)


def invalidate_derived_caches():
    global CACHE_EPOCH
    CACHE_EPOCH += 1
```

Baseline: 1.568 million M elems/s.

## Fuse int8 linear GEMM with residual add, LayerNorm and output quantization

Adds a fused int8 linear + residual + LayerNorm + quantize kernel, with optional split-K workspace, and moves the LN body into a shared header so both paths can reuse it. It is enabled by default in the dense→LayerNorm paths, so the GEMM output no longer round-trips through HBM before normalization. The measured workload is a standalone activation fake-quant, which likely never reaches this path. The fusion also adds row-reduction complexity to the GEMM epilogue and split-K synchronization.

```diff
diff --git a/include/tq_hip.h b/include/tq_hip.h
--- a/include/tq_hip.h
+++ b/include/tq_hip.h
@@ -114,6 +114,16 @@
                             const float* x_zero_float, int x_n_bits, float x_eps, const float* w_delta,
                             uint64_t w_n_params, float w_eps, const tq_quantizer* q_dense,
                             const tq_quantizer* q_sum, const tq_quantizer* q_out, tq_stream_t stream);
+int tq_linear_i8_layernorm_fwd(const int8_t* x_idx, const int8_t* w_idx, const int32_t* w_rowsum, const float* bias,
+                               const float* residual, const float* ln_weight, const float* ln_bias, float ln_eps,
+                               void* y, int8_t* y_idx, int y_dtype, uint64_t M, uint64_t N, uint64_t K,
+                               const float* x_delta, const float* x_zero_float, int x_n_bits, float x_eps,
+                               const float* w_delta, uint64_t w_n_params, float w_eps, const tq_quantizer* q_dense,
+                               const tq_quantizer* q_sum, const tq_quantizer* q_out, void* workspace,
+                               size_t workspace_bytes, uint32_t split_k, tq_stream_t stream);
+size_t tq_linear_i8_layernorm_workspace_bytes(uint64_t M, uint64_t N, uint64_t K, uint32_t split_k);
+int tq_linear_i8_layernorm_plan(uint64_t M, uint64_t N, uint64_t K);
+
 int tq_linear_i8_nonorm_grouped_fwd(const int8_t* x_idx, const int8_t* w_idx, const int32_t* w_rowsum, const float* bias,
                                     const float* nn_weight, const float* nn_bias, void* y, int8_t* y_idx, int y_dtype,
                                     uint64_t M, uint64_t N, uint64_t K, const float* x_delta, const float* x_zero_float,
diff --git a/transformer-quantization_amd/csrc/tq_fused_ln.hip b/transformer-quantization_amd/csrc/tq_fused_ln.hip
--- a/transformer-quantization_amd/csrc/tq_fused_ln.hip
+++ b/transformer-quantization_amd/csrc/tq_fused_ln.hip
@@ -2,294 +2,9 @@
 
 #include "tq_device.h"
 #include "tq_host.h"
+#include "tq_ln_body.h"
 
 namespace tq {
-
-struct FusedQ {
-  QP p;
-  int on;
-  float rcp;
-};
-
-__device__ __forceinline__ FusedQ make_fq(const QP& p, int on) {
-  FusedQ f = {QP{1.f, 0.f, 0.f, 0.f}, on, 1.f};
-  if (on) { f.p = p; f.rcp = guarded_rcp(f.p.scale); }
-  return f;
-}
-__device__ __forceinline__ FusedQ make_fq(const tq_quantizer& q, int on) { return make_fq(on ? make_qp(q, 0) : QP{1.f, 0.f, 0.f, 0.f}, on); }
-
-__device__ __forceinline__ float index_q(float v, const FusedQ& q) {
-  return clamp_nanprop(rne_quot1(v, q.p.scale, q.rcp) + q.p.zp, q.p.lo, q.p.hi);
-}
-
-__device__ __forceinline__ float apply_q(float v, const FusedQ& q) {
-  return q.on ? q_dequant(index_q(v, q), q.p) : v;
-}
-
-template <int CTRL>
-__device__ __forceinline__ float dpp_f32(float v) {
-  return __builtin_bit_cast(float, __builtin_amdgcn_update_dpp(0, __builtin_bit_cast(int, v), CTRL, 0xF, 0xF, true));
-}
-template <int LPR>
-__device__ __forceinline__ float group_sum(float v) {
-  static_assert(LPR >= 4 && LPR <= 64 && (LPR & (LPR - 1)) == 0, "LPR");
-  v += dpp_f32<0xB1>(v);
-  v += dpp_f32<0x4E>(v);
-  if (LPR >= 8) v += dpp_f32<0x141>(v);
-  if (LPR >= 16) v += dpp_f32<0x140>(v);
-  if (LPR >= 32) v += __builtin_bit_cast(float, __builtin_amdgcn_ds_swizzle(__builtin_bit_cast(int, v), 0x401F));
-  if (LPR >= 64) v += __shfl_xor(v, 32, 64);
-  return v;
-}
-
-template <int LPR>
-__device__ __forceinline__ float group_max(float v) {
-  v = max_raw(v, dpp_f32<0xB1>(v));
-  v = max_raw(v, dpp_f32<0x4E>(v));
-  if (LPR >= 8) v = max_raw(v, dpp_f32<0x141>(v));
-  if (LPR >= 16) v = max_raw(v, dpp_f32<0x140>(v));
-  if (LPR >= 32) v = max_raw(v, __builtin_bit_cast(float, __builtin_amdgcn_ds_swizzle(__builtin_bit_cast(int, v), 0x401F)));
-  if (LPR >= 64) v = max_raw(v, __shfl_xor(v, 32, 64));
-  return v;
-}
-
-struct FusedF {
-  QF f;
-  int on;
-};
-__device__ __forceinline__ FusedF make_ff(const QP& p, int on) {
-  FusedF r;
-  r.on = on;
-  r.f = make_qf(on ? p : QP{1.f, 0.f, 0.f, 1.f});
-  return r;
-}
-__device__ __forceinline__ f32x2 apply_f2(f32x2 v, const FusedF& q) { return q.on ? qf_fake_quant2(v, q.f) : v; }
-
-struct EmbArgs {
-  const int64_t *a_rows, *a2_rows, *r_rows;
-  const u32x4* a2;
-  uint64_t a_n, a2_n, r_n;
-  int32_t* bad;
-};
-
-template <int DT, int LPR, int NV, bool EMB>
-__device__ __forceinline__ void ln_load_row(const u32x4* __restrict__ a, const u32x4* __restrict__ r, const EmbArgs& emb, int nt,
-                                            int lane, uint64_t row, u32x4 (&pa)[NV], u32x4 (&pr)[NV], u32x4 (&pa2)[EMB ? NV : 1]) {
-  constexpr int V = Store<DT>::kVec;
-  constexpr uint32_t d = LPR * NV * V;
-  if (EMB) {
-    bool bad = false;
-    auto pick = [&bad](const int64_t* ids, uint64_t row_, uint64_t n) {
-      const int64_t id = ids[row_];
-      const bool out = id < 0 || (uint64_t)id >= n;
-      bad = bad || out;
-      return out ? (uint64_t)0 : (uint64_t)id;
-    };
-    const uint64_t oa = pick(emb.a_rows, row, emb.a_n) * (d / V) + lane;
-    const uint64_t o2 = pick(emb.a2_rows, row, emb.a2_n) * (d / V) + lane;
-    const uint64_t orr = pick(emb.r_rows, row, emb.r_n) * (d / V) + lane;
-#pragma unroll
-    for (int v = 0; v < NV; ++v) { pa[v] = a[oa + v * LPR]; pa2[v] = emb.a2[o2 + v * LPR]; pr[v] = r[orr + v * LPR]; }
-    if (bad) {
-      const u32x4 nan4 = {0x7fc00000u, 0x7fc00000u, 0x7fc00000u, 0x7fc00000u};
-#pragma unroll
-      for (int v = 0; v < NV; ++v) pa[v] = nan4;
-      if (lane == 0 && emb.bad) __hip_atomic_store(emb.bad, 1, __ATOMIC_RELAXED, __HIP_MEMORY_SCOPE_SYSTEM);
-    }
-    return;
-  }
-  const uint64_t o = row * (d / V) + lane;
-  if (nt) {
-#pragma unroll
-    for (int v = 0; v < NV; ++v) { pa[v] = ld_stream(a + o + v * LPR); pr[v] = ld_stream(r + o + v * LPR); }
-  } else {
-#pragma unroll
-    for (int v = 0; v < NV; ++v) { pa[v] = a[o + v * LPR]; pr[v] = r[o + v * LPR]; }
-  }
-}
-
-struct TailQ {
-  QP p1, p2, p3;
-};
-
-template <int DT, int LPR, int NV, bool IDX, bool FAST, bool ALLON, bool AFF, bool EMB>
-__device__ __forceinline__ void res_ln_body(const u32x4* __restrict__ a, const u32x4* __restrict__ r,
-                                            u32x4* __restrict__ y, int8_t* __restrict__ y_idx, uint64_t rows,
-                                            const float* s_w, const float* s_b,
-                                            float ln_eps, const TailQ& tq, int on1_, int on2_, int on3_, int nt, uint32_t iters,
-                                            const EmbArgs& emb, u32x4 (&va)[NV], u32x4 (&vr)[NV], u32x4 (&va2)[EMB ? NV : 1]) {
-  constexpr bool affine_only = AFF;
-  const int on1 = ALLON ? 1 : on1_, on2 = ALLON ? 1 : on2_, on3 = ALLON ? 1 : on3_;
-  constexpr int V = Store<DT>::kVec;
-  constexpr int H = V / 2;
-  constexpr int RPB = kBlock / LPR;
-  constexpr uint32_t d = LPR * NV * V;
-  const FusedF f1 = make_ff(tq.p1, on1), f2 = make_ff(tq.p2, on2), f3 = make_ff(tq.p3, on3);
-  const FusedQ g1 = make_fq(tq.p1, on1), g2 = make_fq(tq.p2, on2), g3 = make_fq(tq.p3, on3);
-  const int lane = threadIdx.x % LPR;
-  const int sub = threadIdx.x / LPR;
-  const float inv_d = 1.0f / (float)d;
-
-  const uint64_t row0 = (uint64_t)blockIdx.x * RPB * iters + sub;
-  u32x4 na[NV], nr[NV];
-  u32x4 na2[EMB ? NV : 1];
-  auto load_row = [&](uint64_t row, u32x4 (&pa)[NV], u32x4 (&pr)[NV], u32x4 (&pa2)[EMB ? NV : 1]) {
-    ln_load_row<DT, LPR, NV, EMB>(a, r, emb, nt, lane, row, pa, pr, pa2);
-  };
-  for (uint32_t it = 0; it < iters; ++it) {
-    const uint64_t row = row0 + (uint64_t)it * RPB;
-    if (row >= rows) break;
-    const uint64_t base = row * (d / V);
-    const uint64_t nrow = row + RPB;
-    if (it + 1 < iters && nrow < rows) load_row(nrow, na, nr, na2);
-    f32x2 u[NV][H];
-    f32x2 s2 = {0.f, 0.f}, s2b = {0.f, 0.f};
-    bool lane_nan = false;
-#pragma unroll
-    for (int v = 0; v < NV; ++v) {
-      float fa[V], fr[V];
-      Store<DT>::unpack(va[v], fa);
-      Store<DT>::unpack(vr[v], fr);
-      if (EMB) {
-        float f2[V];
-        Store<DT>::unpack(va2[v], f2);
-#pragma unroll
-        for (int k = 0; k < V; ++k) fa[k] = fa[k] + f2[k];
-      }
-      if (FAST) {
-        f32x2 t[H];
-#pragma unroll
-        for (int j = 0; j < H; ++j) t[j] = f32x2{fa[2 * j], fa[2 * j + 1]};
-        if (ALLON) qf_fake_quant2_n_signed_zero<H>(t, f1.f);
-        else if (f1.on) qf_fake_quant2_n<H>(t, f1.f);
-#pragma unroll
-        for (int j = 0; j < H; ++j) t[j] = t[j] + f32x2{fr[2 * j], fr[2 * j + 1]};
-        if (ALLON) qf_fake_quant2_n_signed_zero<H>(t, f2.f);
-        else if (f2.on) qf_fake_quant2_n<H>(t, f2.f);
-        if (affine_only) {
-#pragma unroll
-          for (int j = 0; j < H; ++j) {
-            t[j].x = __builtin_isunordered(fa[2 * j], fr[2 * j]) ? __builtin_nanf("") : t[j].x;
-            t[j].y = __builtin_isunordered(fa[2 * j + 1], fr[2 * j + 1]) ? __builtin_nanf("") : t[j].y;
-          }
-        } else {
-#pragma unroll
-          for (int j = 0; j < H; ++j)
-            lane_nan = lane_nan || __builtin_isunordered(fa[2 * j], fr[2 * j]) ||
-                       __builtin_isunordered(fa[2 * j + 1], fr[2 * j + 1]);
-        }
-#pragma unroll
-        for (int j = 0; j < H; ++j) u[v][j] = t[j];
-      } else {
-#pragma unroll
-        for (int j = 0; j < H; ++j)
-          u[v][j] = f32x2{apply_q(apply_q(fa[2 * j], g1) + fr[2 * j], g2),
-                          apply_q(apply_q(fa[2 * j + 1], g1) + fr[2 * j + 1], g2)};
-      }
-      if (!affine_only) {
-#pragma unroll
-        for (int j = 0; j < H; ++j) {
-          if (j & 1) s2b = s2b + u[v][j];
-          else s2 = s2 + u[v][j];
-        }
-      }
-    }
-    s2 = s2 + s2b;
-    float mean = 0.0f, rstd = 1.0f;
-    bool row_nan = false;
-    if (!affine_only) {
-      mean = group_sum<LPR>(s2.x + s2.y) * inv_d;
-      const f32x2 m2 = {mean, mean};
-      f32x2 ssa = {0.f, 0.f}, ssb = {0.f, 0.f};
-#pragma unroll
-      for (int v = 0; v < NV; ++v)
-#pragma unroll
-        for (int j = 0; j < H; ++j) {
-          const f32x2 c = u[v][j] - m2;
-          if ((v * H + j) & 1) ssb = __builtin_elementwise_fma(c, c, ssb);
-          else ssa = __builtin_elementwise_fma(c, c, ssa);
-        }
-      const f32x2 ss2 = ssa + ssb;
-      rstd = 1.0f / sqrtf(group_sum<LPR>(ss2.x + ss2.y) * inv_d + ln_eps);
-      if (FAST) {
-        const uint64_t m = __ballot(lane_nan);
-        const uint64_t grp = LPR == 64 ? ~0ull : (((1ull << (LPR % 64)) - 1) << ((threadIdx.x & 63) / LPR * LPR));
-        if (m & grp) { mean = __builtin_nanf(""); row_nan = true; }
-      }
-    }
-    const f32x2 m2 = {mean, mean}, r2 = {rstd, rstd};
-    u32x4 packed[NV];
-#pragma unroll
-    for (int v = 0; v < NV; ++v) {
-      float o[V];
-      struct alignas(V) { int8_t e[V]; } oi;
-      f32x2 t[H];
-#pragma unroll
-      for (int j = 0; j < H; ++j) {
-        const uint32_t c = (v * LPR + lane) * V + 2 * j;
-        const f32x2 wv = *reinterpret_cast<const f32x2*>(s_w + c), bv = *reinterpret_cast<const f32x2*>(s_b + c);
-        t[j] = (u[v][j] - m2) * r2 * wv + bv;
-      }
-      if (f3.on) {
-        if (FAST) {
-          f32x2 h[H];
-          qf_round2_n<H>(t, f3.f, h);
-#pragma unroll
-          for (int j = 0; j < H; ++j) {
-            if (IDX) {
-              oi.e[2 * j] = (int8_t)((int)(h[j].x + f3.f.zp) - 128);
-              oi.e[2 * j + 1] = (int8_t)((int)(h[j].y + f3.f.zp) - 128);
-            }
-            const f32x2 yq = qf_dequant2(h[j], f3.f);
-            if (affine_only) {
-              t[j].x = (t[j].x != t[j].x) ? t[j].x : yq.x;
-              t[j].y = (t[j].y != t[j].y) ? t[j].y : yq.y;
-            } else {
-              t[j] = yq;
-            }
-          }
-        } else {
-#pragma unroll
-          for (int j = 0; j < H; ++j) {
-            const float x0 = index_q(t[j].x, g3), x1 = index_q(t[j].y, g3);
-            if (IDX) {
-              oi.e[2 * j] = (int8_t)((int)x0 - 128);
-              oi.e[2 * j + 1] = (int8_t)((int)x1 - 128);
-            }
-            t[j] = f32x2{q_dequant(x0, g3.p), q_dequant(x1, g3.p)};
-          }
-        }
-      }
-#pragma unroll
-      for (int j = 0; j < H; ++j) { o[2 * j] = t[j].x; o[2 * j + 1] = t[j].y; }
-      packed[v] = Store<DT>::pack(o);
-      if (IDX) *reinterpret_cast<decltype(oi)*>(y_idx + (base + v * LPR + lane) * V) = oi;
-    }
-    if (nt) {
-#pragma unroll
-      for (int v = 0; v < NV; ++v) st_stream(y + base + v * LPR + lane, packed[v]);
-    } else {
-#pragma unroll
-      for (int v = 0; v < NV; ++v) y[base + v * LPR + lane] = packed[v];
-    }
-    if (FAST && !affine_only && f3.on && __ballot(row_nan)) {
-      if (row_nan) {
-        float nanv[V];
-#pragma unroll
-        for (int e = 0; e < V; ++e) nanv[e] = __builtin_nanf("");
-        const u32x4 pn = Store<DT>::pack(nanv);
-#pragma unroll
-        for (int v = 0; v < NV; ++v) y[base + v * LPR + lane] = pn;
-      }
-    }
-#pragma unroll
-    for (int v = 0; v < NV; ++v) { va[v] = na[v]; vr[v] = nr[v]; }
-    if (EMB) {
-#pragma unroll
-      for (int v = 0; v < NV; ++v) va2[v] = na2[v];
-    }
-  }
-}
 
 template <int DT, int LPR, int NV, bool IDX, bool AFF, bool EMB = false>
 __global__ __launch_bounds__(kBlock) void res_ln_quant_k(const u32x4* __restrict__ a, const u32x4* __restrict__ r,
@@ -328,12 +43,13 @@
   if (on1) fast = fast && make_qf(tq.p1).ok;
   if (on2) fast = fast && make_qf(tq.p2).ok;
   if (on3) fast = fast && make_qf(tq.p3).ok;
+  const GlobalRows<DT, LPR, NV, EMB> src{a, r, emb, nt, (int)(threadIdx.x % LPR)};
   if (fast && on1 && on2 && on3)
-    res_ln_body<DT, LPR, NV, IDX, true, true, AFF, EMB>(a, r, y, y_idx, rows, s_w, s_b, ln_eps, tq, 1, 1, 1, nt, iters, emb, va, vr, va2);
+    res_ln_body<DT, LPR, NV, IDX, true, true, AFF, EMB>(src, blockIdx.x, y, y_idx, rows, s_w, s_b, ln_eps, tq, 1, 1, 1, nt, iters, va, vr, va2);
   else if (fast)
-    res_ln_body<DT, LPR, NV, IDX, true, false, AFF, EMB>(a, r, y, y_idx, rows, s_w, s_b, ln_eps, tq, on1, on2, on3, nt, iters, emb, va, vr, va2);
+    res_ln_body<DT, LPR, NV, IDX, true, false, AFF, EMB>(src, blockIdx.x, y, y_idx, rows, s_w, s_b, ln_eps, tq, on1, on2, on3, nt, iters, va, vr, va2);
   else
-    res_ln_body<DT, LPR, NV, IDX, false, false, AFF, EMB>(a, r, y, y_idx, rows, s_w, s_b, ln_eps, tq, on1, on2, on3, nt, iters, emb, va, vr, va2);
+    res_ln_body<DT, LPR, NV, IDX, false, false, AFF, EMB>(src, blockIdx.x, y, y_idx, rows, s_w, s_b, ln_eps, tq, on1, on2, on3, nt, iters, va, vr, va2);
 }
 
 template <int DT>
diff --git a/transformer-quantization_amd/csrc/tq_linear_args.h b/transformer-quantization_amd/csrc/tq_linear_args.h
--- /dev/null
+++ b/transformer-quantization_amd/csrc/tq_linear_args.h
@@ -0,0 +1,96 @@
+#pragma once
+
+#include "tq_device.h"
+#include "tq_host.h"
+
+namespace tq {
+
+typedef int v4i __attribute__((ext_vector_type(4)));
+
+enum { ACT_NONE = 0, ACT_RELU = 1, ACT_GELU = 2, ACT_TANH = 3 };
+
+struct LinArgs {
+  const int8_t* x;
+  const int8_t* w;
+  const int32_t* w_rowsum;
+  const float* bias;
+  void* y;
+  int8_t* y_idx;
+  uint32_t M, N, K;
+  const float* x_delta;
+  const float* x_zero_float;
+  float x_eps;
+  int x_n_bits;
+  const float* w_delta;
+  uint32_t w_n_params;
+  float w_eps;
+  int act;
+  int has_q;
+  tq_quantizer q_out;
+  tq_quantizer q_out1, q_out2;
+  uint32_t group_cols;
+  int fast_epi;
+  int dbg;
+  int tail;
+  const float* residual;
+  const float* nn_w;
+  const float* nn_b;
+  tq_quantizer q_t1, q_t2;
+  int on_t1, on_t2;
+  tq_quantizer q_t2b, q_t2c;
+  int split_out;
+  const float* stair;
+  uint32_t stair_bins;
+};
+
+__device__ __forceinline__ void input_scale_shift(float dx, float zx, float x_eps, int x_n_bits, float& sx, int& shift) {
+  sx = dx < x_eps ? x_eps : dx;
+  const int z = (int)clamp_nanprop(rintf(zx), 0.0f, grid_top(x_n_bits));
+  shift = 128 - z;
+}
+
+struct LinShape {
+  uint32_t mn, k;
+  const char* rule;
+};
+constexpr LinShape kAnyShape{32, 64, "M,N % 32, K % 64"};
+constexpr LinShape kTiledShape{64, 128, "M, N % 64, K % 128"};
+constexpr LinShape kGroupedShape{64, 128, "M % 64, K % 128"};
+
+static int lin_args(LinArgs& a, const char* who, const LinShape& s, const int8_t* x, const int8_t* w, const int32_t* w_rowsum,
+                    const float* bias, void* y, int8_t* y_idx, bool need_y, int y_dtype, uint64_t M, uint64_t N, uint64_t K,
+                    const float* x_delta, const float* x_zero_float, int x_n_bits, float x_eps, const float* w_delta,
+                    uint64_t w_n_params, float w_eps, int act) {
+  TQ_REQUIRE(x && w && w_rowsum && (need_y ? y != nullptr : y || y_idx) && x_delta && x_zero_float && w_delta, "%s: NULL pointer", who);
+  TQ_REQUIRE(y_dtype == TQ_F32 || y_dtype == TQ_BF16, "%s: y dtype must be fp32 or bf16", who);
+  TQ_REQUIRE(M % s.mn == 0 && N % s.mn == 0 && K % s.k == 0 && K >= s.k && K <= 16384 && M < (1u << 31) && N < (1u << 31),
+             "%s: unsupported shape M=%llu N=%llu K=%llu (%s)", who, (unsigned long long)M, (unsigned long long)N,
+             (unsigned long long)K, s.rule);
+  TQ_REQUIRE(x_n_bits >= 1 && x_n_bits <= 8, "%s: input quantizer must have <= 8 bits", who);
+  TQ_REQUIRE(w_n_params == 1 || w_n_params == N, "%s: weight scales must be per-tensor or per-output-channel", who);
+  TQ_REQUIRE(act >= ACT_NONE && act <= ACT_TANH, "%s: unknown activation %d", who, act);
+  TQ_REQUIRE(aligned16(x) && aligned16(w) && (y == nullptr || aligned16(y)), "%s: 16-byte alignment required", who);
+  a.x = x; a.w = w; a.w_rowsum = w_rowsum; a.bias = bias; a.y = y; a.y_idx = y_idx;
+  a.M = (uint32_t)M; a.N = (uint32_t)N; a.K = (uint32_t)K;
+  a.x_delta = x_delta; a.x_zero_float = x_zero_float; a.x_eps = x_eps; a.x_n_bits = x_n_bits;
+  a.w_delta = w_delta; a.w_n_params = (uint32_t)w_n_params; a.w_eps = w_eps; a.act = act;
+  a.group_cols = (uint32_t)N;
+  return TQ_OK;
+}
+
+static int check_y_idx(const char* who, const int8_t* y_idx, const tq_quantizer* q, bool groups = false) {
+  if (y_idx == nullptr || (q != nullptr && !q->symmetric && q->n_bits <= 8)) return TQ_OK;
+  return set_error(TQ_EINVAL, groups ? "%s: y_idx needs asymmetric <= 8-bit output quantizers"
+                                     : "%s: y_idx needs an asymmetric <= 8-bit output quantizer", who);
+}
+
+static int quantizer_slot(const char* who, const char* what, const tq_quantizer* q, uint64_t n, tq_quantizer& slot, int& on) {
+  on = q != nullptr;
+  if (q == nullptr) return TQ_OK;
+  if (int e = check_quantizer(q, n, who)) return e;
+  TQ_REQUIRE(q->n_params == 1, "%s: per-tensor %s only", who, what);
+  slot = *q;
+  return TQ_OK;
+}
+
+}
diff --git a/transformer-quantization_amd/csrc/tq_linear_i8.hip b/transformer-quantization_amd/csrc/tq_linear_i8.hip
--- a/transformer-quantization_amd/csrc/tq_linear_i8.hip
+++ b/transformer-quantization_amd/csrc/tq_linear_i8.hip
@@ -3,12 +3,9 @@
 
 #include "tq_device.h"
 #include "tq_host.h"
+#include "tq_linear_args.h"
 
 namespace tq {
-
-typedef int v4i __attribute__((ext_vector_type(4)));
-
-enum { ACT_NONE = 0, ACT_RELU = 1, ACT_GELU = 2, ACT_TANH = 3 };
 
 __device__ __forceinline__ float apply_act(float v, int act) {
   switch (act) {
@@ -18,40 +15,6 @@
     default: return v;
   }
 }
-
-struct LinArgs {
-  const int8_t* x;
-  const int8_t* w;
-  const int32_t* w_rowsum;
-  const float* bias;
-  void* y;
-  int8_t* y_idx;
-  uint32_t M, N, K;
-  const float* x_delta;
-  const float* x_zero_float;
-  float x_eps;
-  int x_n_bits;
-  const float* w_delta;
-  uint32_t w_n_params;
-  float w_eps;
-  int act;
-  int has_q;
-  tq_quantizer q_out;
-  tq_quantizer q_out1, q_out2;
-  uint32_t group_cols;
-  int fast_epi;
-  int dbg;
-  int tail;
-  const float* residual;
-  const float* nn_w;
-  const float* nn_b;
-  tq_quantizer q_t1, q_t2;
-  int on_t1, on_t2;
-  tq_quantizer q_t2b, q_t2c;
-  int split_out;
-  const float* stair;
-  uint32_t stair_bins;
-};
 
 struct StairRef {
   const u32x2* tab;
@@ -475,9 +438,7 @@
 template <bool WITH_TAIL, bool SEL = false>
 __device__ __forceinline__ EpiCtx epilogue_finish(const LinArgs& p, const EpiRaw& w) {
   EpiCtx c;
-  c.sx = w.dx < p.x_eps ? p.x_eps : w.dx;
-  const int zx = (int)clamp_nanprop(rintf(w.zx), 0.0f, grid_top(p.x_n_bits));
-  c.shift = 128 - zx;
+  input_scale_shift(w.dx, w.zx, p.x_eps, p.x_n_bits, c.sx, c.shift);
   c.qo = QP{1.f, 0.f, 0.f, 0.f};
   if (p.has_q) c.qo = qp_from_raw<SEL>(w.qsel, w.qo);
   c.qf = make_qf(c.qo);
@@ -1308,49 +1269,6 @@
   return a.tail ? launch_linear_t<TQ_BF16, true>(a, st) : launch_linear_t<TQ_BF16, false>(a, st);
 }
 
-struct LinShape {
-  uint32_t mn, k;
-  const char* rule;
-};
-constexpr LinShape kAnyShape{32, 64, "M,N % 32, K % 64"};
-constexpr LinShape kTiledShape{64, 128, "M, N % 64, K % 128"};
-constexpr LinShape kGroupedShape{64, 128, "M % 64, K % 128"};
-
-static int lin_args(LinArgs& a, const char* who, const LinShape& s, const int8_t* x, const int8_t* w, const int32_t* w_rowsum,
-                    const float* bias, void* y, int8_t* y_idx, bool need_y, int y_dtype, uint64_t M, uint64_t N, uint64_t K,
-                    const float* x_delta, const float* x_zero_float, int x_n_bits, float x_eps, const float* w_delta,
-                    uint64_t w_n_params, float w_eps, int act) {
-  TQ_REQUIRE(x && w && w_rowsum && (need_y ? y != nullptr : y || y_idx) && x_delta && x_zero_float && w_delta, "%s: NULL pointer", who);
-  TQ_REQUIRE(y_dtype == TQ_F32 || y_dtype == TQ_BF16, "%s: y dtype must be fp32 or bf16", who);
-  TQ_REQUIRE(M % s.mn == 0 && N % s.mn == 0 && K % s.k == 0 && K >= s.k && K <= 16384 && M < (1u << 31) && N < (1u << 31),
-             "%s: unsupported shape M=%llu N=%llu K=%llu (%s)", who, (unsigned long long)M, (unsigned long long)N,
-             (unsigned long long)K, s.rule);
-  TQ_REQUIRE(x_n_bits >= 1 && x_n_bits <= 8, "%s: input quantizer must have <= 8 bits", who);
-  TQ_REQUIRE(w_n_params == 1 || w_n_params == N, "%s: weight scales must be per-tensor or per-output-channel", who);
-  TQ_REQUIRE(act >= ACT_NONE && act <= ACT_TANH, "%s: unknown activation %d", who, act);
-  TQ_REQUIRE(aligned16(x) && aligned16(w) && (y == nullptr || aligned16(y)), "%s: 16-byte alignment required", who);
-  a.x = x; a.w = w; a.w_rowsum = w_rowsum; a.bias = bias; a.y = y; a.y_idx = y_idx;
-  a.M = (uint32_t)M; a.N = (uint32_t)N; a.K = (uint32_t)K;
-  a.x_delta = x_delta; a.x_zero_float = x_zero_float; a.x_eps = x_eps; a.x_n_bits = x_n_bits;
-  a.w_delta = w_delta; a.w_n_params = (uint32_t)w_n_params; a.w_eps = w_eps; a.act = act;
-  a.group_cols = (uint32_t)N;
-  return TQ_OK;
-}
-
-static int check_y_idx(const char* who, const int8_t* y_idx, const tq_quantizer* q, bool groups = false) {
-  if (y_idx == nullptr || (q != nullptr && !q->symmetric && q->n_bits <= 8)) return TQ_OK;
-  return set_error(TQ_EINVAL, groups ? "%s: y_idx needs asymmetric <= 8-bit output quantizers"
-                                     : "%s: y_idx needs an asymmetric <= 8-bit output quantizer", who);
-}
-
-static int quantizer_slot(const char* who, const char* what, const tq_quantizer* q, uint64_t n, tq_quantizer& slot, int& on) {
-  on = q != nullptr;
-  if (q == nullptr) return TQ_OK;
-  if (int e = check_quantizer(q, n, who)) return e;
-  TQ_REQUIRE(q->n_params == 1, "%s: per-tensor %s only", who, what);
-  slot = *q;
-  return TQ_OK;
-}
 
 static int nonorm_quantizers(LinArgs& a, const char* who, uint64_t n, const tq_quantizer* q_dense, const tq_quantizer* q_sum,
                              const tq_quantizer* q_out) {
diff --git a/transformer-quantization_amd/csrc/tq_linear_ln_i8.hip b/transformer-quantization_amd/csrc/tq_linear_ln_i8.hip
--- /dev/null
+++ b/transformer-quantization_amd/csrc/tq_linear_ln_i8.hip
@@ -0,0 +1,355 @@
+#include <algorithm>
+#include <type_traits>
+
+#include "tq_device.h"
+#include "tq_host.h"
+#include "tq_linear_args.h"
+#include "tq_ln_body.h"
+
+namespace tq {
+
+constexpr int kPanelN = 768;
+constexpr int kPanelM = 16;
+constexpr int kPanelNT = kPanelN / 4 / 16;
+constexpr int kPieceBytes = 16 * 128;
+constexpr int kRingBytes = 4 * kPanelNT * kPieceBytes;
+constexpr int kPanelPitch = kPanelN * 4 + 16;
+constexpr uint32_t kMaxSplitK = 8;
+static_assert(kPanelM * kPanelPitch <= kRingBytes, "the fp32 panel reuses the ring");
+
+struct LinLnArgs {
+  const int8_t* x;
+  const int8_t* w;
+  const int32_t* w_rowsum;
+  const float* bias;
+  const float* residual;
+  const float* ln_w;
+  const float* ln_b;
+  float* y;
+  int8_t* y_idx;
+  uint32_t M, K;
+  const float* x_delta;
+  const float* x_zero_float;
+  float x_eps;
+  int x_n_bits;
+  const float* w_delta;
+  uint32_t w_n_params;
+  float w_eps, ln_eps;
+  tq_quantizer q1, q2, q3;
+  int on1, on2, on3;
+  uint32_t sk;
+  uint32_t* ctr;
+  v4i* part;
+};
+
+static inline size_t panel_lds_bytes(uint32_t kp) {
+  return (size_t)kRingBytes + (size_t)kp * kPanelM + 2 * kPanelN * 4 + 3 * kPanelN * 4 + 16;
+}
+
+#define TQ_GLDS16(gp, lp)                                                                         \
+  __builtin_amdgcn_global_load_lds((const __attribute__((address_space(1))) void*)(gp),           \
+                                   (__attribute__((address_space(3))) void*)(lp), 16, 0, 0)
+
+template <int N>
+__device__ __forceinline__ void vm_wait_but() {
+  asm volatile("s_waitcnt vmcnt(%0)" ::"n"(N) : "memory");
+}
+__device__ __forceinline__ void lds_reads_done() { asm volatile("s_waitcnt lgkmcnt(0)" ::: "memory"); }
+__device__ __forceinline__ void pin_vec(u32x4& v) { asm volatile("" : "+v"(v)); }
+__device__ __forceinline__ void pin_f(float& v) { asm volatile("" : "+v"(v)); }
+__device__ __forceinline__ void pin_i(int& v) { asm volatile("" : "+v"(v)); }
+
+__device__ __forceinline__ void store_through(v4i* p, v4i v) {
+  asm volatile("global_store_dwordx4 %0, %1, off sc1\n\ts_nop 1" ::"v"(p), "v"(v) : "memory");
+}
+__device__ __forceinline__ v4i load_through(const v4i* p) {
+  const uint64_t* q = reinterpret_cast<const uint64_t*>(p);
+  const uint64_t lo = __hip_atomic_load(q, __ATOMIC_RELAXED, __HIP_MEMORY_SCOPE_AGENT);
+  const uint64_t hi = __hip_atomic_load(q + 1, __ATOMIC_RELAXED, __HIP_MEMORY_SCOPE_AGENT);
+  return v4i{(int)(uint32_t)lo, (int)(uint32_t)(lo >> 32), (int)(uint32_t)hi, (int)(uint32_t)(hi >> 32)};
+}
+
+struct PanelRows {
+  const int8_t* panel;
+  const u32x4* __restrict__ r;
+  uint64_t row_base;
+  int lane;
+  __device__ __forceinline__ void load(uint64_t row, u32x4 (&pa)[3], u32x4 (&pr)[3], u32x4 (&)[1]) const {
+    const int8_t* prow = panel + (row - row_base) * kPanelPitch;
+    const uint64_t o = row * (kPanelN / 4) + lane;
+#pragma unroll
+    for (int v = 0; v < 3; ++v) {
+      pa[v] = *reinterpret_cast<const u32x4*>(prow + (v * 64 + lane) * 16);
+      pr[v] = r[o + v * 64];
+    }
+  }
+};
+
+template <bool IDX>
+__global__ __launch_bounds__(kBlock) void linear_ln_i8_k(LinLnArgs p) {
+  constexpr int NT = kPanelNT, LPR = 64, NV = 3, RPB = kBlock / LPR;
+  extern __shared__ __attribute__((aligned(1024))) int8_t lds[];
+  prefetch_kernarg<sizeof(LinLnArgs)>();
+  const int tid = threadIdx.x, lane = tid & 63, wave = __builtin_amdgcn_readfirstlane(tid >> 6);
+  const uint32_t sk = p.sk, kp = p.K / sk, nkp = kp / 128;
+  const uint32_t panel = blockIdx.x / sk, ks = blockIdx.x - panel * sk;
+  const uint32_t m0 = panel * kPanelM, k0 = ks * kp;
+  int8_t* ring = lds + wave * (NT * kPieceBytes);
+  int8_t* xl = lds + kRingBytes;
+  float* s_w = reinterpret_cast<float*>(xl + (size_t)kp * kPanelM);
+  float* s_b = s_w + kPanelN;
+  float* cst = s_b + kPanelN;
+  uint32_t* s_flag = reinterpret_cast<uint32_t*>(cst + 3 * kPanelN);
+  const int r16 = lane & 15, kg = lane >> 4;
+  const int swz = (r16 >> 1) & 7;
+  const int off[2] = {r16 * 128 + ((kg ^ swz) << 4), r16 * 128 + (((4 + kg) ^ swz) << 4)};
+
+  const u32x4* rv = reinterpret_cast<const u32x4*>(p.residual);
+  u32x4 vr[NV];
+  {
+    const uint64_t o = (uint64_t)(m0 + tid / LPR) * (kPanelN / 4) + (tid % LPR);
+#pragma unroll
+    for (int v = 0; v < NV; ++v) vr[v] = rv[o + v * LPR];
+  }
+  float c_dw[3], c_b[3], a_w[3], a_b[3];
+  int c_rs[3];
+#pragma unroll
+  for (int i = 0; i < 3; ++i) {
+    const uint32_t c = tid + i * kBlock;
+    c_dw[i] = p.w_delta[p.w_n_params == 1 ? 0 : c];
+    c_b[i] = p.bias ? p.bias[c] : 0.0f;
+    c_rs[i] = p.w_rowsum[c];
+    a_w[i] = p.ln_w[c];
+    a_b[i] = p.ln_b[c];
+  }
+  float dx = p.x_delta[0], zx = p.x_zero_float[0];
+  QRaw w1 = load_qraw(p.q1, 0, p.ln_w), w2 = load_qraw(p.q2, 0, p.ln_w), w3 = load_qraw(p.q3, 0, p.ln_w);
+
+  const int lrow = lane >> 3;
+  const int lchunk[2] = {(lane & 7) ^ ((lrow >> 1) & 7), (lane & 7) ^ (((8 + lrow) >> 1) & 7)};
+  {
+    const int8_t* xs0 = p.x + (size_t)(m0 + lrow) * p.K + k0 + lchunk[0] * 16;
+    const int8_t* xs1 = p.x + (size_t)(m0 + 8 + lrow) * p.K + k0 + lchunk[1] * 16;
+    for (uint32_t t = wave; t < nkp; t += 4) {
+      TQ_GLDS16(xs0 + t * 128, xl + t * kPieceBytes);
+      TQ_GLDS16(xs1 + t * 128, xl + t * kPieceBytes + 1024);
+    }
+  }
+  const int8_t* ws0 = p.w + (size_t)(wave * (NT * 16) + lrow) * p.K + k0 + lchunk[0] * 16;
+  const int8_t* ws1 = p.w + (size_t)(wave * (NT * 16) + 8 + lrow) * p.K + k0 + lchunk[1] * 16;
+  const size_t piece_stride = (size_t)16 * p.K;
+  auto issue = [&](int i, uint32_t kb) {
+    TQ_GLDS16(ws0 + i * piece_stride + kb * 128, ring + i * kPieceBytes);
+    TQ_GLDS16(ws1 + i * piece_stride + kb * 128, ring + i * kPieceBytes + 1024);
+  };
+#pragma unroll
+  for (int i = 0; i < NT; ++i) issue(i, 0);
+
+#pragma unroll
+  for (int v = 0; v < NV; ++v) pin_vec(vr[v]);
+#pragma unroll
+  for (int i = 0; i < 3; ++i) { pin_f(c_dw[i]); pin_f(c_b[i]); pin_i(c_rs[i]); pin_f(a_w[i]); pin_f(a_b[i]); }
+  dx = pinned_uniform(dx);
+  zx = pinned_uniform(zx);
+  qraw_arrived(w1); qraw_arrived(w2); qraw_arrived(w3);
+  vm_wait_but<0>();
+  __syncthreads();
+
+  v4i acc[NT];
+#pragma unroll
+  for (int i = 0; i < NT; ++i) acc[i] = v4i{0, 0, 0, 0};
+
+  v4i fw0 = *reinterpret_cast<const v4i*>(ring + off[0]), fw1 = *reinterpret_cast<const v4i*>(ring + off[1]);
+  v4i fx0 = *reinterpret_cast<const v4i*>(xl + off[0]), fx1 = *reinterpret_cast<const v4i*>(xl + off[1]);
+  lds_reads_done();
+  auto slab = [&](uint32_t kb, auto last_tag) {
+    constexpr bool LAST = decltype(last_tag)::value;
+#pragma unroll
+    for (int i = 0; i < NT; ++i) {
+      if (!LAST) issue(i, kb + 1);
+      v4i nw0 = fw0, nw1 = fw1, nx0 = fx0, nx1 = fx1;
+      if (i + 1 < NT) {
+        if (LAST) {
+          switch (i) {
+            case 0: vm_wait_but<20>(); break; case 1: vm_wait_but<18>(); break; case 2: vm_wait_but<16>(); break;
+            case 3: vm_wait_but<14>(); break; case 4: vm_wait_but<12>(); break; case 5: vm_wait_but<10>(); break;
+            case 6: vm_wait_but<8>(); break; case 7: vm_wait_but<6>(); break; case 8: vm_wait_but<4>(); break;
+            case 9: vm_wait_but<2>(); break; default: vm_wait_but<0>(); break;
+          }
+        } else {
+          vm_wait_but<2 * (NT - 1)>();
+        }
+        nw0 = *reinterpret_cast<const v4i*>(ring + (i + 1) * kPieceBytes + off[0]);
+        nw1 = *reinterpret_cast<const v4i*>(ring + (i + 1) * kPieceBytes + off[1]);
+      } else if (!LAST) {
+        vm_wait_but<2 * (NT - 1)>();
+        nw0 = *reinterpret_cast<const v4i*>(ring + off[0]);
+        nw1 = *reinterpret_cast<const v4i*>(ring + off[1]);
+        nx0 = *reinterpret_cast<const v4i*>(xl + (kb + 1) * kPieceBytes + off[0]);
+        nx1 = *reinterpret_cast<const v4i*>(xl + (kb + 1) * kPieceBytes + off[1]);
+      }
+      acc[i] = __builtin_amdgcn_mfma_i32_16x16x64_i8(fw0, fx0, acc[i], 0, 0, 0);
+      acc[i] = __builtin_amdgcn_mfma_i32_16x16x64_i8(fw1, fx1, acc[i], 0, 0, 0);
+      lds_reads_done();
+      fw0 = nw0; fw1 = nw1; fx0 = nx0; fx1 = nx1;
+    }
+  };
+  for (uint32_t kb = 0; kb + 1 < nkp; ++kb) slab(kb, std::false_type{});
+  slab(nkp - 1, std::true_type{});
+
+  if (sk > 1) {
+    v4i* mine = p.part + ((size_t)(panel * sk + ks) * 4 + wave) * (NT * 64) + lane;
+#pragma unroll
+    for (int i = 0; i < NT; ++i) store_through(mine + i * 64, acc[i]);
+    vm_wait_but<0>();
+    __syncthreads();
+    if (tid == 0) *s_flag = __hip_atomic_fetch_add(p.ctr + panel, 1u, __ATOMIC_RELAXED, __HIP_MEMORY_SCOPE_AGENT);
+    __syncthreads();
+    if (*s_flag != sk - 1) return;
+    if (tid == 0) __hip_atomic_store(p.ctr + panel, 0u, __ATOMIC_RELAXED, __HIP_MEMORY_SCOPE_AGENT);
+    for (uint32_t s = 0; s < sk; ++s) {
+      if (s == ks) continue;
+      const v4i* theirs = p.part + ((size_t)(panel * sk + s) * 4 + wave) * (NT * 64) + lane;
+      v4i t[NT];
+#pragma unroll
+      for (int i = 0; i < NT; ++i) t[i] = load_through(theirs + i * 64);
+#pragma unroll
+      for (int i = 0; i < NT; ++i) acc[i] = acc[i] + t[i];
+    }
+  } else {
+    __syncthreads();
+  }
+
+  float sx;
+  int shift;
+  input_scale_shift(dx, zx, p.x_eps, p.x_n_bits, sx, shift);
+#pragma unroll
+  for (int i = 0; i < 3; ++i) {
+    const uint32_t c = tid + i * kBlock;
+    cst[c] = sx * (c_dw[i] < p.w_eps ? p.w_eps : c_dw[i]);
+    cst[kPanelN + c] = c_b[i];
+    reinterpret_cast<int*>(cst)[2 * kPanelN + c] = c_rs[i] * shift;
+    s_w[c] = a_w[i];
+    s_b[c] = a_b[i];
+  }
+  __syncthreads();
+  int8_t* pan = lds;
+#pragma unroll
+  for (int i = 0; i < NT; ++i) {
+    const int col = wave * (NT * 16) + i * 16 + kg * 4;
+    const f32x4 s4 = *reinterpret_cast<const f32x4*>(cst + col);
+    const f32x4 b4 = *reinterpret_cast<const f32x4*>(cst + kPanelN + col);
+    const v4i r4 = *reinterpret_cast<const v4i*>(cst + 2 * kPanelN + col);
+    const v4i t = acc[i] + r4;
+    const f32x4 v = __builtin_convertvector(t, f32x4) * s4 + b4;
+    *reinterpret_cast<f32x4*>(pan + r16 * kPanelPitch + col * 4) = v;
+  }
+  __syncthreads();
+
+  const QP none = {1.f, 0.f, 0.f, 0.f};
+  const TailQ tq = {p.on1 ? qp_from_raw(p.q1, w1) : none, p.on2 ? qp_from_raw(p.q2, w2) : none, p.on3 ? qp_from_raw(p.q3, w3) : none};
+  bool fast = true;
+  if (p.on1) fast = fast && make_qf(tq.p1).ok;
+  if (p.on2) fast = fast && make_qf(tq.p2).ok;
+  if (p.on3) fast = fast && make_qf(tq.p3).ok;
+  const PanelRows src{pan, rv, m0, tid % LPR};
+  u32x4 va[NV], dummy[1];
+#pragma unroll
+  for (int v = 0; v < NV; ++v)
+    va[v] = *reinterpret_cast<const u32x4*>(pan + (tid / LPR) * kPanelPitch + (v * LPR + tid % LPR) * 16);
+  u32x4* yv = reinterpret_cast<u32x4*>(p.y);
+  constexpr uint32_t iters = kPanelM / RPB;
+  if (fast && p.on1 && p.on2 && p.on3)
+    res_ln_body<TQ_F32, LPR, NV, IDX, true, true, false, false>(src, panel, yv, p.y_idx, p.M, s_w, s_b, p.ln_eps, tq, 1, 1, 1, 0, iters, va, vr, dummy);
+  else if (fast)
+    res_ln_body<TQ_F32, LPR, NV, IDX, true, false, false, false>(src, panel, yv, p.y_idx, p.M, s_w, s_b, p.ln_eps, tq, p.on1, p.on2, p.on3, 0, iters, va, vr, dummy);
+  else
+    res_ln_body<TQ_F32, LPR, NV, IDX, false, false, false, false>(src, panel, yv, p.y_idx, p.M, s_w, s_b, p.ln_eps, tq, p.on1, p.on2, p.on3, 0, iters, va, vr, dummy);
+}
+
+static bool split_ok(uint32_t sk, uint64_t K) { return sk >= 1 && sk <= kMaxSplitK && (K / 128) % sk == 0; }
+
+static uint32_t auto_split_k(uint64_t M, uint64_t K) {
+  const uint64_t panels = M / kPanelM;
+  uint32_t best = 1;
+  for (uint32_t sk = 2; sk <= kMaxSplitK; ++sk)
+    if (split_ok(sk, K) && panels * sk <= 256) best = sk;
+  return best;
+}
+
+static size_t counters_bytes(uint64_t M) { return (size_t)ceil_div(M / kPanelM * 4, 256) * 256; }
+
+}
+
+using namespace tq;
+
+extern "C" int tq_linear_i8_layernorm_plan(uint64_t M, uint64_t N, uint64_t K) {
+  if (N != (uint64_t)kPanelN || M == 0 || M % kPanelM != 0 || K % 128 != 0 || K < 128 || K > 16384) return 0;
+  if (K > (uint64_t)tuning("TQ_LIN_LN_MAX_K", 1024)) return 0;
+  if (M <= (uint64_t)tuning("TQ_LIN_LN_MIN_M", 2048) || M > (uint64_t)tuning("TQ_LIN_LN_MAX_M", 4096)) return 0;
+  return (int)auto_split_k(M, K);
+}
+
+extern "C" size_t tq_linear_i8_layernorm_workspace_bytes(uint64_t M, uint64_t N, uint64_t K, uint32_t split_k) {
+  if (N != (uint64_t)kPanelN || M % kPanelM != 0 || K % 128 != 0 || K < 128) return 0;
+  const uint32_t sk = split_k ? split_k : auto_split_k(M, K);
+  if (!split_ok(sk, K) || sk == 1) return 0;
+  return counters_bytes(M) + (size_t)(M / kPanelM) * sk * 4 * kPanelNT * 64 * sizeof(v4i);
+}
+
+extern "C" int tq_linear_i8_layernorm_fwd(const int8_t* x_idx, const int8_t* w_idx, const int32_t* w_rowsum, const float* bias,
+                                          const float* residual, const float* ln_weight, const float* ln_bias, float ln_eps,
+                                          void* y, int8_t* y_idx, int y_dtype, uint64_t M, uint64_t N, uint64_t K,
+                                          const float* x_delta, const float* x_zero_float, int x_n_bits, float x_eps,
+                                          const float* w_delta, uint64_t w_n_params, float w_eps,
+                                          const tq_quantizer* q_dense, const tq_quantizer* q_sum, const tq_quantizer* q_out,
+                                          void* workspace, size_t workspace_bytes, uint32_t split_k, tq_stream_t stream) {
+  const char* who = "tq_linear_i8_layernorm_fwd";
+  if (M == 0 || N == 0) return TQ_OK;
+  if (y_dtype != TQ_F32) return set_error(TQ_EUNSUPPORTED, "%s: fp32 output only", who);
+  if (N != (uint64_t)kPanelN) return set_error(TQ_EUNSUPPORTED, "%s: built for N = %d output features, got %llu", who, kPanelN, (unsigned long long)N);
+  if (M % kPanelM != 0 || K % 128 != 0) return set_error(TQ_EUNSUPPORTED, "%s: M %% 16 == 0 and K %% 128 == 0 required", who);
+  for (const tq_quantizer* q : {q_dense, q_sum, q_out})
+    if (q != nullptr && q->n_params != 1) return set_error(TQ_EUNSUPPORTED, "%s: per-tensor quantizers only", who);
+  LinArgs a{};
+  if (int e = lin_args(a, who, LinShape{16, 128, "M % 16, N = 768, K % 128"}, x_idx, w_idx, w_rowsum, bias, y, y_idx, true, y_dtype, M, N, K,
+                       x_delta, x_zero_float, x_n_bits, x_eps, w_delta, w_n_params, w_eps, ACT_NONE))
+    return e;
+  TQ_REQUIRE(residual && ln_weight && ln_bias, "%s: NULL pointer", who);
+  TQ_REQUIRE(aligned16(residual), "%s: 16-byte alignment required", who);
+  if (int e = check_y_idx(who, y_idx, q_out)) return e;
+  TQ_REQUIRE(y_idx == nullptr || (reinterpret_cast<uintptr_t>(y_idx) & 7u) == 0, "%s: y_idx needs 8-byte alignment", who);
+  LinLnArgs k{};
+  if (int e = quantizer_slot(who, "quantizers", q_dense, M * N, k.q1, k.on1)) return e;
+  if (int e = quantizer_slot(who, "quantizers", q_sum, M * N, k.q2, k.on2)) return e;
+  if (int e = quantizer_slot(who, "quantizers", q_out, M * N, k.q3, k.on3)) return e;
+  const uint32_t sk = split_k ? split_k : auto_split_k(M, K);
+  TQ_REQUIRE(split_ok(sk, K), "%s: split_k = %u must be 1..%u and divide K / 128 = %llu", who, sk, kMaxSplitK, (unsigned long long)(K / 128));
+  const size_t lds = panel_lds_bytes((uint32_t)(K / sk));
+  if (lds > 160 * 1024)
+    return set_error(TQ_EUNSUPPORTED, "%s: a [16, %llu] input panel does not fit the LDS of a workgroup (raise split_k)", who, (unsigned long long)(K / sk));
+  const size_t need = sk > 1 ? counters_bytes(M) + (size_t)(M / kPanelM) * sk * 4 * kPanelNT * 64 * sizeof(v4i) : 0;
+  TQ_REQUIRE(sk == 1 || (workspace != nullptr && workspace_bytes >= need && aligned16(workspace)),
+             "%s: split_k = %u needs %zu bytes of 16-byte aligned workspace (tq_linear_i8_layernorm_workspace_bytes)", who, sk, need);
+  k.x = a.x; k.w = a.w; k.w_rowsum = a.w_rowsum; k.bias = a.bias; k.residual = residual; k.ln_w = ln_weight; k.ln_b = ln_bias;
+  k.y = static_cast<float*>(y); k.y_idx = y_idx; k.M = a.M; k.K = a.K;
+  k.x_delta = a.x_delta; k.x_zero_float = a.x_zero_float; k.x_eps = a.x_eps; k.x_n_bits = a.x_n_bits;
+  k.w_delta = a.w_delta; k.w_n_params = a.w_n_params; k.w_eps = a.w_eps; k.ln_eps = ln_eps;
+  k.sk = sk;
+  k.ctr = static_cast<uint32_t*>(workspace);
+  k.part = sk > 1 ? reinterpret_cast<v4i*>(static_cast<char*>(workspace) + counters_bytes(M)) : nullptr;
+  static bool attr_set[64] = {};
+  int dev = 0;
+  if (hipGetDevice(&dev) != hipSuccess || dev < 0 || dev >= 64) dev = -1;
+  if (dev < 0 || !attr_set[dev]) {
+    if (hipFuncSetAttribute(reinterpret_cast<const void*>(linear_ln_i8_k<true>), hipFuncAttributeMaxDynamicSharedMemorySize, 160 * 1024) != hipSuccess ||
+        hipFuncSetAttribute(reinterpret_cast<const void*>(linear_ln_i8_k<false>), hipFuncAttributeMaxDynamicSharedMemorySize, 160 * 1024) != hipSuccess)
+      return set_error(TQ_ELAUNCH, "%s: cannot reserve 160 KB of LDS", who);
+    if (dev >= 0) attr_set[dev] = true;
+  }
+  const dim3 grid((unsigned)((M / kPanelM) * sk));
+  hipStream_t st = static_cast<hipStream_t>(stream);
+  if (y_idx != nullptr) hipLaunchKernelGGL(linear_ln_i8_k<true>, grid, dim3(kBlock), lds, st, k);
+  else                  hipLaunchKernelGGL(linear_ln_i8_k<false>, grid, dim3(kBlock), lds, st, k);
+  return check_launch("linear_ln_i8_k");
+}
diff --git a/transformer-quantization_amd/csrc/tq_ln_body.h b/transformer-quantization_amd/csrc/tq_ln_body.h
--- /dev/null
+++ b/transformer-quantization_amd/csrc/tq_ln_body.h
@@ -0,0 +1,301 @@
+#pragma once
+
+#include "tq_device.h"
+
+namespace tq {
+
+struct FusedQ {
+  QP p;
+  int on;
+  float rcp;
+};
+
+__device__ __forceinline__ FusedQ make_fq(const QP& p, int on) {
+  FusedQ f = {QP{1.f, 0.f, 0.f, 0.f}, on, 1.f};
+  if (on) { f.p = p; f.rcp = guarded_rcp(f.p.scale); }
+  return f;
+}
+__device__ __forceinline__ FusedQ make_fq(const tq_quantizer& q, int on) { return make_fq(on ? make_qp(q, 0) : QP{1.f, 0.f, 0.f, 0.f}, on); }
+
+__device__ __forceinline__ float index_q(float v, const FusedQ& q) {
+  return clamp_nanprop(rne_quot1(v, q.p.scale, q.rcp) + q.p.zp, q.p.lo, q.p.hi);
+}
+
+__device__ __forceinline__ float apply_q(float v, const FusedQ& q) {
+  return q.on ? q_dequant(index_q(v, q), q.p) : v;
+}
+
+template <int CTRL>
+__device__ __forceinline__ float dpp_f32(float v) {
+  return __builtin_bit_cast(float, __builtin_amdgcn_update_dpp(0, __builtin_bit_cast(int, v), CTRL, 0xF, 0xF, true));
+}
+template <int LPR>
+__device__ __forceinline__ float group_sum(float v) {
+  static_assert(LPR >= 4 && LPR <= 64 && (LPR & (LPR - 1)) == 0, "LPR");
+  v += dpp_f32<0xB1>(v);
+  v += dpp_f32<0x4E>(v);
+  if (LPR >= 8) v += dpp_f32<0x141>(v);
+  if (LPR >= 16) v += dpp_f32<0x140>(v);
+  if (LPR >= 32) v += __builtin_bit_cast(float, __builtin_amdgcn_ds_swizzle(__builtin_bit_cast(int, v), 0x401F));
+  if (LPR >= 64) v += __shfl_xor(v, 32, 64);
+  return v;
+}
+
+template <int LPR>
+__device__ __forceinline__ float group_max(float v) {
+  v = max_raw(v, dpp_f32<0xB1>(v));
+  v = max_raw(v, dpp_f32<0x4E>(v));
+  if (LPR >= 8) v = max_raw(v, dpp_f32<0x141>(v));
+  if (LPR >= 16) v = max_raw(v, dpp_f32<0x140>(v));
+  if (LPR >= 32) v = max_raw(v, __builtin_bit_cast(float, __builtin_amdgcn_ds_swizzle(__builtin_bit_cast(int, v), 0x401F)));
+  if (LPR >= 64) v = max_raw(v, __shfl_xor(v, 32, 64));
+  return v;
+}
+
+struct FusedF {
+  QF f;
+  int on;
+};
+__device__ __forceinline__ FusedF make_ff(const QP& p, int on) {
+  FusedF r;
+  r.on = on;
+  r.f = make_qf(on ? p : QP{1.f, 0.f, 0.f, 1.f});
+  return r;
+}
+__device__ __forceinline__ f32x2 apply_f2(f32x2 v, const FusedF& q) { return q.on ? qf_fake_quant2(v, q.f) : v; }
+
+struct EmbArgs {
+  const int64_t *a_rows, *a2_rows, *r_rows;
+  const u32x4* a2;
+  uint64_t a_n, a2_n, r_n;
+  int32_t* bad;
+};
+
+template <int DT, int LPR, int NV, bool EMB>
+__device__ __forceinline__ void ln_load_row(const u32x4* __restrict__ a, const u32x4* __restrict__ r, const EmbArgs& emb, int nt,
+                                            int lane, uint64_t row, u32x4 (&pa)[NV], u32x4 (&pr)[NV], u32x4 (&pa2)[EMB ? NV : 1]) {
+  constexpr int V = Store<DT>::kVec;
+  constexpr uint32_t d = LPR * NV * V;
+  if (EMB) {
+    bool bad = false;
+    auto pick = [&bad](const int64_t* ids, uint64_t row_, uint64_t n) {
+      const int64_t id = ids[row_];
+      const bool out = id < 0 || (uint64_t)id >= n;
+      bad = bad || out;
+      return out ? (uint64_t)0 : (uint64_t)id;
+    };
+    const uint64_t oa = pick(emb.a_rows, row, emb.a_n) * (d / V) + lane;
+    const uint64_t o2 = pick(emb.a2_rows, row, emb.a2_n) * (d / V) + lane;
+    const uint64_t orr = pick(emb.r_rows, row, emb.r_n) * (d / V) + lane;
+#pragma unroll
+    for (int v = 0; v < NV; ++v) { pa[v] = a[oa + v * LPR]; pa2[v] = emb.a2[o2 + v * LPR]; pr[v] = r[orr + v * LPR]; }
+    if (bad) {
+      const u32x4 nan4 = {0x7fc00000u, 0x7fc00000u, 0x7fc00000u, 0x7fc00000u};
+#pragma unroll
+      for (int v = 0; v < NV; ++v) pa[v] = nan4;
+      if (lane == 0 && emb.bad) __hip_atomic_store(emb.bad, 1, __ATOMIC_RELAXED, __HIP_MEMORY_SCOPE_SYSTEM);
+    }
+    return;
+  }
+  const uint64_t o = row * (d / V) + lane;
+  if (nt) {
+#pragma unroll
+    for (int v = 0; v < NV; ++v) { pa[v] = ld_stream(a + o + v * LPR); pr[v] = ld_stream(r + o + v * LPR); }
+  } else {
+#pragma unroll
+    for (int v = 0; v < NV; ++v) { pa[v] = a[o + v * LPR]; pr[v] = r[o + v * LPR]; }
+  }
+}
+
+struct TailQ {
+  QP p1, p2, p3;
+};
+
+template <int DT, int LPR, int NV, bool EMB>
+struct GlobalRows {
+  const u32x4* __restrict__ a;
+  const u32x4* __restrict__ r;
+  const EmbArgs& emb;
+  int nt, lane;
+  __device__ __forceinline__ void load(uint64_t row, u32x4 (&pa)[NV], u32x4 (&pr)[NV], u32x4 (&pa2)[EMB ? NV : 1]) const {
+    ln_load_row<DT, LPR, NV, EMB>(a, r, emb, nt, lane, row, pa, pr, pa2);
+  }
+};
+
+template <int DT, int LPR, int NV, bool IDX, bool FAST, bool ALLON, bool AFF, bool EMB, class SRC>
+__device__ __forceinline__ void res_ln_body(const SRC& src, uint32_t blk,
+                                            u32x4* __restrict__ y, int8_t* __restrict__ y_idx, uint64_t rows,
+                                            const float* s_w, const float* s_b,
+                                            float ln_eps, const TailQ& tq, int on1_, int on2_, int on3_, int nt, uint32_t iters,
+                                            u32x4 (&va)[NV], u32x4 (&vr)[NV], u32x4 (&va2)[EMB ? NV : 1]) {
+  constexpr bool affine_only = AFF;
+  const int on1 = ALLON ? 1 : on1_, on2 = ALLON ? 1 : on2_, on3 = ALLON ? 1 : on3_;
+  constexpr int V = Store<DT>::kVec;
+  constexpr int H = V / 2;
+  constexpr int RPB = kBlock / LPR;
+  constexpr uint32_t d = LPR * NV * V;
+  const FusedF f1 = make_ff(tq.p1, on1), f2 = make_ff(tq.p2, on2), f3 = make_ff(tq.p3, on3);
+  const FusedQ g1 = make_fq(tq.p1, on1), g2 = make_fq(tq.p2, on2), g3 = make_fq(tq.p3, on3);
+  const int lane = threadIdx.x % LPR;
+  const int sub = threadIdx.x / LPR;
+  const float inv_d = 1.0f / (float)d;
+
+  const uint64_t row0 = (uint64_t)blk * RPB * iters + sub;
+  u32x4 na[NV], nr[NV];
+  u32x4 na2[EMB ? NV : 1];
+  for (uint32_t it = 0; it < iters; ++it) {
+    const uint64_t row = row0 + (uint64_t)it * RPB;
+    if (row >= rows) break;
+    const uint64_t base = row * (d / V);
+    const uint64_t nrow = row + RPB;
+    if (it + 1 < iters && nrow < rows) src.load(nrow, na, nr, na2);
+    f32x2 u[NV][H];
+    f32x2 s2 = {0.f, 0.f}, s2b = {0.f, 0.f};
+    bool lane_nan = false;
+#pragma unroll
+    for (int v = 0; v < NV; ++v) {
+      float fa[V], fr[V];
+      Store<DT>::unpack(va[v], fa);
+      Store<DT>::unpack(vr[v], fr);
+      if (EMB) {
+        float f2[V];
+        Store<DT>::unpack(va2[v], f2);
+#pragma unroll
+        for (int k = 0; k < V; ++k) fa[k] = fa[k] + f2[k];
+      }
+      if (FAST) {
+        f32x2 t[H];
+#pragma unroll
+        for (int j = 0; j < H; ++j) t[j] = f32x2{fa[2 * j], fa[2 * j + 1]};
+        if (ALLON) qf_fake_quant2_n_signed_zero<H>(t, f1.f);
+        else if (f1.on) qf_fake_quant2_n<H>(t, f1.f);
+#pragma unroll
+        for (int j = 0; j < H; ++j) t[j] = t[j] + f32x2{fr[2 * j], fr[2 * j + 1]};
+        if (ALLON) qf_fake_quant2_n_signed_zero<H>(t, f2.f);
+        else if (f2.on) qf_fake_quant2_n<H>(t, f2.f);
+        if (affine_only) {
+#pragma unroll
+          for (int j = 0; j < H; ++j) {
+            t[j].x = __builtin_isunordered(fa[2 * j], fr[2 * j]) ? __builtin_nanf("") : t[j].x;
+            t[j].y = __builtin_isunordered(fa[2 * j + 1], fr[2 * j + 1]) ? __builtin_nanf("") : t[j].y;
+          }
+        } else {
+#pragma unroll
+          for (int j = 0; j < H; ++j)
+            lane_nan = lane_nan || __builtin_isunordered(fa[2 * j], fr[2 * j]) ||
+                       __builtin_isunordered(fa[2 * j + 1], fr[2 * j + 1]);
+        }
+#pragma unroll
+        for (int j = 0; j < H; ++j) u[v][j] = t[j];
+      } else {
+#pragma unroll
+        for (int j = 0; j < H; ++j)
+          u[v][j] = f32x2{apply_q(apply_q(fa[2 * j], g1) + fr[2 * j], g2),
+                          apply_q(apply_q(fa[2 * j + 1], g1) + fr[2 * j + 1], g2)};
+      }
+      if (!affine_only) {
+#pragma unroll
+        for (int j = 0; j < H; ++j) {
+          if (j & 1) s2b = s2b + u[v][j];
+          else s2 = s2 + u[v][j];
+        }
+      }
+    }
+    s2 = s2 + s2b;
+    float mean = 0.0f, rstd = 1.0f;
+    bool row_nan = false;
+    if (!affine_only) {
+      mean = group_sum<LPR>(s2.x + s2.y) * inv_d;
+      const f32x2 m2 = {mean, mean};
+      f32x2 ssa = {0.f, 0.f}, ssb = {0.f, 0.f};
+#pragma unroll
+      for (int v = 0; v < NV; ++v)
+#pragma unroll
+        for (int j = 0; j < H; ++j) {
+          const f32x2 c = u[v][j] - m2;
+          if ((v * H + j) & 1) ssb = __builtin_elementwise_fma(c, c, ssb);
+          else ssa = __builtin_elementwise_fma(c, c, ssa);
+        }
+      const f32x2 ss2 = ssa + ssb;
+      rstd = 1.0f / sqrtf(group_sum<LPR>(ss2.x + ss2.y) * inv_d + ln_eps);
+      if (FAST) {
+        const uint64_t m = __ballot(lane_nan);
+        const uint64_t grp = LPR == 64 ? ~0ull : (((1ull << (LPR % 64)) - 1) << ((threadIdx.x & 63) / LPR * LPR));
+        if (m & grp) { mean = __builtin_nanf(""); row_nan = true; }
+      }
+    }
+    const f32x2 m2 = {mean, mean}, r2 = {rstd, rstd};
+    u32x4 packed[NV];
+#pragma unroll
+    for (int v = 0; v < NV; ++v) {
+      float o[V];
+      struct alignas(V) { int8_t e[V]; } oi;
+      f32x2 t[H];
+#pragma unroll
+      for (int j = 0; j < H; ++j) {
+        const uint32_t c = (v * LPR + lane) * V + 2 * j;
+        const f32x2 wv = *reinterpret_cast<const f32x2*>(s_w + c), bv = *reinterpret_cast<const f32x2*>(s_b + c);
+        t[j] = (u[v][j] - m2) * r2 * wv + bv;
+      }
+      if (f3.on) {
+        if (FAST) {
+          f32x2 h[H];
+          qf_round2_n<H>(t, f3.f, h);
+#pragma unroll
+          for (int j = 0; j < H; ++j) {
+            if (IDX) {
+              oi.e[2 * j] = (int8_t)((int)(h[j].x + f3.f.zp) - 128);
+              oi.e[2 * j + 1] = (int8_t)((int)(h[j].y + f3.f.zp) - 128);
+            }
+            const f32x2 yq = qf_dequant2(h[j], f3.f);
+            if (affine_only) {
+              t[j].x = (t[j].x != t[j].x) ? t[j].x : yq.x;
+              t[j].y = (t[j].y != t[j].y) ? t[j].y : yq.y;
+            } else {
+              t[j] = yq;
+            }
+          }
+        } else {
+#pragma unroll
+          for (int j = 0; j < H; ++j) {
+            const float x0 = index_q(t[j].x, g3), x1 = index_q(t[j].y, g3);
+            if (IDX) {
+              oi.e[2 * j] = (int8_t)((int)x0 - 128);
+              oi.e[2 * j + 1] = (int8_t)((int)x1 - 128);
+            }
+            t[j] = f32x2{q_dequant(x0, g3.p), q_dequant(x1, g3.p)};
+          }
+        }
+      }
+#pragma unroll
+      for (int j = 0; j < H; ++j) { o[2 * j] = t[j].x; o[2 * j + 1] = t[j].y; }
+      packed[v] = Store<DT>::pack(o);
+      if (IDX) *reinterpret_cast<decltype(oi)*>(y_idx + (base + v * LPR + lane) * V) = oi;
+    }
+    if (nt) {
+#pragma unroll
+      for (int v = 0; v < NV; ++v) st_stream(y + base + v * LPR + lane, packed[v]);
+    } else {
+#pragma unroll
+      for (int v = 0; v < NV; ++v) y[base + v * LPR + lane] = packed[v];
+    }
+    if (FAST && !affine_only && f3.on && __ballot(row_nan)) {
+      if (row_nan) {
+        float nanv[V];
+#pragma unroll
+        for (int e = 0; e < V; ++e) nanv[e] = __builtin_nanf("");
+        const u32x4 pn = Store<DT>::pack(nanv);
+#pragma unroll
+        for (int v = 0; v < NV; ++v) y[base + v * LPR + lane] = pn;
+      }
+    }
+#pragma unroll
+    for (int v = 0; v < NV; ++v) { va[v] = na[v]; vr[v] = nr[v]; }
+    if (EMB) {
+#pragma unroll
+      for (int v = 0; v < NV; ++v) va2[v] = na2[v];
+    }
+  }
+}
+
+}
diff --git a/transformer-quantization_amd/quantization/_hip.py b/transformer-quantization_amd/quantization/_hip.py
--- a/transformer-quantization_amd/quantization/_hip.py
+++ b/transformer-quantization_amd/quantization/_hip.py
@@ -91,6 +91,10 @@
                                     _vp, _vp, _vp, _QP, _QP, _QP, _vp, _vp, _int, _u64, _u64, _u64, _u64, _vp]),
     'tq_linear_i8_nonorm_fwd': (_int, [_vp, _vp, _vp, _vp, _vp, _vp, _vp, _vp, _vp, _int, _u64, _u64, _u64, _vp, _vp, _int, _f,
                                        _vp, _u64, _f, _QP, _QP, _QP, _vp]),
+    'tq_linear_i8_layernorm_fwd': (_int, [_vp, _vp, _vp, _vp, _vp, _vp, _vp, _f, _vp, _vp, _int, _u64, _u64, _u64, _vp, _vp, _int,
+                                          _f, _vp, _u64, _f, _QP, _QP, _QP, _vp, _sz, C.c_uint32, _vp]),
+    'tq_linear_i8_layernorm_workspace_bytes': (_sz, [_u64, _u64, _u64, C.c_uint32]),
+    'tq_linear_i8_layernorm_plan': (_int, [_u64, _u64, _u64]),
     'tq_ffn_chain_i8_nonorm_fwd': (_int, [_vp, _vp, _vp, _int, _f, _vp, _vp, _u64, _vp, _vp, _int, _u64, _u64, _u64, _u64, _vp]),
     'tq_linear_i8_nonorm_grouped_fwd': (_int, [_vp, _vp, _vp, _vp, _vp, _vp, _vp, _vp, _int, _u64, _u64, _u64, _vp, _vp, _int, _f, _vp,
                                                _f, _u64, C.POINTER(_QP), C.POINTER(_QP), _vp]),
@@ -299,6 +303,8 @@
         self._qdesc_cache = {}
         self._ws_bytes = {}
         self._counters = {}
+        self._lin_ln_ws = {}
+        self._lin_ln_plan = {}
         self._calib_tensor_addr = None
 
     def _workspace(self, device, nbytes):
@@ -655,6 +661,45 @@
             _ptr(nn_b.detach().float().contiguous()), _ptr(y), _ptr(y_idx), _DTYPES[out_dtype], M, N, K, _ptr(x_q[0]),
             _ptr(x_q[1]), int(x_q[2]), float(x_q[3]), _ptr(w_delta), w_delta.numel(), float(w_eps), refs[0], refs[1],
             refs[2], _stream())
+        _check(rc, self.lib)
+        return (y, y_idx) if want_idx else y
+
+    def linear_i8_layernorm_plan(self, M, N, K):
+        key = (M, N, K)
+        sk = self._lin_ln_plan.get(key)
+        if sk is None:
+            sk = self._lin_ln_plan[key] = int(self.lib.tq_linear_i8_layernorm_plan(M, N, K))
+        return sk
+
+    def _linear_ln_workspace(self, device, M, N, K, split_k):
+        nbytes = int(self.lib.tq_linear_i8_layernorm_workspace_bytes(M, N, K, split_k))
+        if nbytes == 0:
+            return None, 0
+        key = (device.index, _stream(), nbytes)
+        ws = self._lin_ln_ws.get(key)
+        if ws is None:
+            ws = self._lin_ln_ws[key] = torch.empty(nbytes, dtype=torch.uint8, device=device)
+            ws[:(M // 16 * 4 + 255) // 256 * 256].zero_()
+        return ws, nbytes
+
+    def linear_i8_layernorm(self, x_idx, w_idx, w_rowsum, bias, residual, ln_w, ln_b, ln_eps, x_q, w_delta, w_eps, q_dense,
+                            q_sum, q_out, want_idx=False, split_k=0):
+        K = x_idx.shape[-1]
+        M = x_idx.numel() // K
+        N = w_idx.shape[0]
+        y = torch.empty(x_idx.shape[:-1] + (N,), dtype=torch.float32, device=x_idx.device)
+        y_idx = torch.empty(y.shape, dtype=torch.int8, device=y.device) if want_idx else None
+        descs = [None if q is None else self._qdesc(*q, 1, 1) for q in (q_dense, q_sum, q_out)]
+        refs = [None if d is None else C.byref(d) for d in descs]
+        residual = residual.detach().float().contiguous()
+        ln_w = ln_w.detach().float().contiguous()
+        ln_b = ln_b.detach().float().contiguous()
+        ws, ws_bytes = self._linear_ln_workspace(x_idx.device, M, N, K, int(split_k))
+        rc = self.lib.tq_linear_i8_layernorm_fwd(
+            _ptr(x_idx), _ptr(w_idx), _ptr(w_rowsum), _ptr(bias), _ptr(residual), _ptr(ln_w), _ptr(ln_b), float(ln_eps),
+            _ptr(y), _ptr(y_idx), _DTYPES[torch.float32], M, N, K, _ptr(x_q[0]), _ptr(x_q[1]), int(x_q[2]), float(x_q[3]),
+            _ptr(w_delta), w_delta.numel(), float(w_eps), refs[0], refs[1], refs[2], _ptr(ws), ws_bytes, int(split_k),
+            _stream())
         _check(rc, self.lib)
         return (y, y_idx) if want_idx else y
 
diff --git a/transformer-quantization_amd/quantization/fused.py b/transformer-quantization_amd/quantization/fused.py
--- a/transformer-quantization_amd/quantization/fused.py
+++ b/transformer-quantization_amd/quantization/fused.py
@@ -91,6 +91,10 @@
         y = _linear_nonorm_i8(dense, layer_norm, x, residual, q1, q2, q3)
         if y is not None:
             return y
+    if not is_nonorm and _gemm is None and not axis:
+        y = _linear_layernorm_i8(dense, layer_norm, residual, q1, q2, q3, x=x)
+        if y is not None:
+            return y
     gemm = _gemm
     if gemm is None and options.int8_active() and hasattr(dense, '_int8_forward'):
         gemm = dense._int8_forward(x, with_output_quantizer=False)
@@ -191,6 +195,10 @@
     mid_idx = intermediate._int8_compute(x, plan1, index_only=True)
     if mid_idx is None:
         return separate()
+    if not _per_column(q1, q2, q3):
+        y = _linear_layernorm_i8(dense, layer_norm, residual, q1, q2, q3, plan=plan2, x_idx=mid_idx)
+        if y is not None:
+            return y
     gemm = dense._int8_compute(None, plan2, x_idx=mid_idx)
     if gemm is None:
         return separate()
@@ -209,6 +217,38 @@
         elif any(p.requires_grad for p in m.parameters()):
             return True
     return False
+
+
+def _linear_layernorm_i8(dense, layer_norm, residual, q1, q2, q3, x=None, plan=None, x_idx=None):
+    if not options.INT8_LINEAR_LAYERNORM or not options.int8_active() or not hasattr(dense, '_int8_plan'):
+        return None
+    be = _hip.backend()
+    if not hasattr(be, 'linear_i8_layernorm'):
+        return None
+    if not be.linear_i8_layernorm_plan(residual.numel() // dense.out_features, dense.out_features, dense.in_features):
+        return None
+    if ('no' in (q1, q2, q3) or _per_column(q1, q2, q3) or residual.dtype != torch.float32 or not _hip.on_device(residual)
+            or len(layer_norm.normalized_shape) != 1 or _needs_autograd(dense, layer_norm, x, residual)):
+        return None
+    if plan is None:
+        plan = dense._int8_plan(x, with_output_quantizer=False)
+    if plan is None or len(plan) > 3 or plan[1] != _hip.ACT_NONE:
+        return None
+    ops = dense._int8_operands(x, plan, x_idx)
+    if ops is None:
+        return None
+    from quantization.autoquant_utils import INT8_STATS
+    arg = lambda q: None if q == 'off' else q
+    ln_w, ln_b = layer_norm.get_params()
+    oq = layer_norm.activation_quantizer.quantizer if q3 != 'off' else None
+    want_idx = oq is not None and not oq.symmetric and oq.n_bits <= 8
+    INT8_STATS['kernel_calls'] += 1
+    out = be.linear_i8_layernorm(ops[0], ops[1], ops[2], ops[3], residual, ln_w, ln_b, layer_norm.eps, ops[4], ops[5], ops[6],
+                                 arg(q1), arg(q2), arg(q3), want_idx=want_idx)
+    y = out[0] if want_idx else out
+    if oq is not None:
+        provenance.tag(y, oq, out[1] if want_idx else None)
+    return y
 
 
 def _linear_nonorm_i8(dense, layer_norm, x, residual, q1, q2, q3):
diff --git a/transformer-quantization_amd/quantization/options.py b/transformer-quantization_amd/quantization/options.py
--- a/transformer-quantization_amd/quantization/options.py
+++ b/transformer-quantization_amd/quantization/options.py
@@ -6,6 +6,8 @@
 INT8_CALIBRATION_MIN_MACS = 1 << 33
 
 INT8_ACT_STAIR = True
+
+INT8_LINEAR_LAYERNORM = True
 
 LOCKSTEP_WEIGHT_SEARCH = True
 
```

After: 1.549 million M elems/s. 0.988x the previous value.
